# claussss/ubisoft-laforge-daft-exprt

Measured on AMD Instinct MI355X. Metric: mel frames/sec (fwd+bwd), higher is better.
Workload: dtype bf16

## Files before the change

include/daft_exprt_hip.h:

```cpp
#ifndef DAFT_EXPRT_HIP_H
#define DAFT_EXPRT_HIP_H

#include <stdint.h>

#ifdef __cplusplus
extern "C" {
#endif

int dx_version(void);
const char* dx_last_error(void);
int dx_prof_enable(int kind, int capacity);
int dx_prof_collect(int kind, int* launches, double* total_ms);

int dx_int_durations(const float* dur, int B, int L, int sampling_rate, int filter_length, int hop_length, int centered,
                     long long* out, long long* totals, int* status);

int dx_pack_dims(int Cout, int Cin, int bf16, int* dims);
int dx_pack_weights(const float* W, void* fwd, void* bwd, int Cout, int Cin, int taps, int bf16, void* stream);
int dx_pack_weights_batched(const void* descs, int n, int bf16, void* stream);
int dx_pack_weights_host(const void* descs, int n, int bf16, void* stream);
int dx_conv_gemm(const void* X, int ldx, const void* Wp, const float* bias, void* Y, int ldy,
                 int B, int N, int Cin, int Cout, int taps, int bf16,
                 int relu, const float* post_scale, const float* post_shift,
                 const void* relu_aux, int ld_aux, int accumulate,
                 const int* lens, int mask_rows, float out_scale, int skip_halo,
                 int x_bf16, int y_bf16, int aux_bf16, const int* rows_exist, void* stream);
int dx_conv_wgrad(const void* dY, int ldy, const void* X, int ldx, float* G,
                  int B, int N, int Cin, int Cout, int taps, const int* lens, int skip_halo,
                  int bf16, int dy_bf16, int x_bf16, float* dbias, const int* rows_exist, void* stream);
typedef struct DxWgradJob {
  const void* dY; const void* X; float* G; float* dbias; const int* lens;
  int ldy, ldx, B, N, Cin, Cout, skip_halo, reserved;
  const int* rows_exist;
} DxWgradJob;
int dx_conv_wgrad_batched(const void* jobs, int njobs, int taps, int dy_bf16, int x_bf16, void* stream);
int dx_unpack_wgrad(const float* G, float* grad, int Cout, int Cin, int taps, int accumulate, void* stream);
int dx_ff_pair(const void* X, int ldx, const void* Wa, const void* Wb, const float* bias_a, const float* bias_b,
               const void* aux, int ld_aux, void* H, int ldh, float* Y, int ldy,
               int B, int N, int F, int relu_mid, int accumulate, const int* lens, int skip_halo, const int* rows_exist, void* stream);
int dx_ff_pair_ln(const void* X, int ldx, const void* Wa, const void* Wb, const float* bias_a, const float* bias_b, void* H, int ldh, float* Z,
                  int B, int N, int F, const int* lens, int skip_halo, const int* rows_exist,
                  const float* res, const float* ln_w, const float* ln_b, const float* film, int ld_film, float* Yln, float* mean, float* rstd,
                  uint64_t seed_pre, float p_pre, const uint64_t* seed_offset, void* hmask, void* stream);
int dx_ff_pair_ln_qkv(const void* X, int ldx, const void* Wa, const void* Wb, const float* bias_a, const float* bias_b, void* H, int ldh, float* Z,
                      int B, int N, int F, const int* lens, int skip_halo, const int* rows_exist,
                      const float* res, const float* ln_w, const float* ln_b, const float* film, int ld_film, float* Yln, float* mean, float* rstd,
                      uint64_t seed_pre, float p_pre, const uint64_t* seed_offset, const void* Wq, const float* bias_q, void* QKV, void* hmask, void* stream);
int dx_ff_pair_lnbwd(const void* X, int ldx, const void* Wa, const void* Wb, const void* aux, int ld_aux, void* H, int ldh, float* Y,
                     int B, int N, int F, const int* lens, int skip_halo,
                     const float* z, const float* mean, const float* rstd, const float* ln_w, const float* ln_b, void* DG, float* dw, float* db,
                     uint64_t seed_pre, float p_pre, const uint64_t* seed_offset, void* stream);
int dx_ff_block_bwd(const float* dY2, const float* z2, const float* mean2, const float* rstd2, const float* ln2_w, const float* ln2_b,
                    const float* film, int ld_film, void* DG2, float* dw2, float* db2, float* dfilm, int ld_dfilm, uint64_t seed2, float p2,
                    const void* Wa, const void* Wb, const void* aux, int ld_aux, void* H, int ldh, float* Y,
                    int B, int N, int F, const int* lens, int skip_halo,
                    const float* z1, const float* mean1, const float* rstd1, const float* ln1_w, const float* ln1_b, void* DG1, float* dw1, float* db1,
                    uint64_t seed1, float p1, const void* Wout_bwd, void* DATT, const uint64_t* seed_offset, const void* hmask,
                    const int* rows_exist, void* stream);
int dx_colsum(const void* X, int ldx, float* out, long rows, int C, int x_bf16, void* stream);

int dx_length_order(const int* lens, int* order, int B, void* stream);
int dx_attention_fwd(const void* qkv, int ld, const int* lens, void* ctx, int ldc, float* lse,
                     int B, int N, int H, int D, uint64_t seed, const uint64_t* seed_offset, float p_drop, int bf16, int qkv_bf16, int ctx_bf16,
                     const int* order, void* stream);
int dx_attention_proj_ln_fwd(const void* qkv, int ld, const int* lens, void* ctx, int ldc, float* lse, int B, int N, int H, int D,
                             uint64_t seed, const uint64_t* seed_offset, float p_drop,
                             const void* Wpack, const float* proj_bias, float* z, const float* res, const float* w, const float* bias,
                             const float* film, int ld_film, float* y, float* mean, float* rstd, uint64_t seed_pre, float p_pre,
                             void* y_bf16_copy, void* stream);
int dx_attention_bwd(const void* qkv, int ld, const void* ctx, const void* dctx, int ldc, const float* lse, float* delta,
                     const int* lens, void* dqkv, int ldg, int B, int N, int H, int D, uint64_t seed, const uint64_t* seed_offset, float p_drop, int bf16,
                     int qkv_bf16, int dqkv_bf16, int ctx_bf16, const int* order, void* stream);

int dx_ln_fwd(void* a, const void* res, const float* w, const float* bias, const float* film, int ld_film,
              const int* lens, int halo, void* y, float* mean, float* rstd, int B, int N, int C,
              uint64_t seed_pre, float p_pre, uint64_t seed_post, float p_post, const uint64_t* seed_offset, int io_bf16, void* y_bf16_copy,
              void* stream);
int dx_film_affine_fwd(const float* gammas, const float* betas, const float* pm, float* film, int B, int nb, int C, void* stream);
int dx_film_affine_bwd(const void* dfilm_ptrs, const float* gammas, const float* betas, const float* pm, float* dgammas, float* dbetas, float* dpm,
                       int B, int nb, int C, void* stream);
int dx_proj_ln_fwd(const void* X, int ldx, const void* Wpack, const float* proj_bias, float* z, const float* res, const float* w, const float* bias,
                   const float* film, int ld_film, const int* lens, int halo, float* y, float* mean, float* rstd, int B, int N,
                   uint64_t seed_pre, float p_pre, const uint64_t* seed_offset, void* y_bf16_copy, void* stream);
int dx_ln_bwd(const void* dy, const void* z, const float* mean, const float* rstd, const float* w, const float* bias,
              const float* film, int ld_film, const int* lens, int halo, void* dz, void* da, float* dw, float* dbias,
              float* dfilm, int ld_dfilm, int B, int N, int C, int relu_mask,
              uint64_t seed_pre, float p_pre, uint64_t seed_post, float p_post, const uint64_t* seed_offset, int io_bf16, void* dg_bf16_copy,
              void* stream);

int dx_add_pos(const float* x, const long* sym, const float* emb, const float* pe, const int* lens, float* out,
               int B, int N, int D, int pe_rows, void* stream);
int dx_mask_rows(const float* in, const int* lens, float* out, int B, int N, int C, void* stream);
int dx_embedding_bwd(const float* dout, const long* sym, const int* lens, float* demb, int B, int N, int D, void* stream);
int dx_accent_sum(const float* prenet, const float* energy, const float* pitch, const float* we, const float* be,
                  const float* wp, const float* bp, const float* pe, const int* lens, float* out,
                  int B, int N, int D, int pe_rows, void* stream);
int dx_scalar_conv_wgrad(const float* dout, int ldd, const float* rowscale, const float* s0, const float* s1, const int* lens,
                         float* dw0, float* db0, float* dw1, float* db1, int B, int N, int D, void* stream);
int dx_mean_pool(const float* x, const int* lens, float* out, int B, int N, int C, void* stream);
int dx_mean_pool_bwd(const float* dout, const int* lens, float* dx, int B, int N, int C, void* stream);
int dx_transpose(const float* in, float* out, int B, int R, int Cc, int accumulate, void* stream);
int dx_relu_bwd(const float* dy, const float* y, float* out, long n, void* stream);
int dx_channel_affine(const void* x, const float* scale, const float* shift, void* out, long rows, int C, int io_bf16, void* stream);
int dx_l2_normalize(const float* x, float* y, int rows, int C, void* stream);
int dx_cross_entropy(const float* logits, const long* target, float* loss, float* dlogits, int B, int S, void* stream);

int dx_duration_scan(const long* dur_int, float* mu, long* totals, int B, int L, void* stream);
int dx_upsample_prep(const float* enc, const float* dur, const float* energy, const float* pitch,
                     const float* wd, const float* bd, const float* we, const float* be, const float* wp, const float* bp,
                     const float* wr, const float* br, const int* lens, float* xs, float* z, float* sigma,
                     int B, int L, int D, void* stream);
int dx_upsample_fwd(const float* xs, const float* mu, const float* sigma, const int* lens, float* weights, float* xup,
                    int B, int L, int T, int D, void* stream);
int dx_upsample_bwd(const float* dxup, const float* xs, const float* mu, const float* sigma, const float* weights, const int* lens,
                    float* dxs, float* dsigma, int B, int L, int T, int D, void* stream);
int dx_upsample_sym_bwd(const float* dxs_in, const float* dsigma, const float* xs, const float* z, const float* dur, const int* lens,
                        const float* wd, const float* bd, const float* wr, float* dxs_out, float* dz, float* dwr, float* dbr,
                        int B, int L, int D, void* stream);

int dx_mel_stats(const float* mel_pred, const float* mel_target, float* ep, float* et, float* l1sum, float* l2sum,
                 int B, int M, int T, void* stream);
int dx_energy_diff(const float* ep, const float* et, const int* lens, float* des, float* esum, int B, int T, const int* rows_exist, void* stream);
int dx_mel_grad(const float* mel_pred, const float* mel_target, const float* ep, const float* des, const int* lens,
                float c_l1, float c_l2, float c_e, int e_per_total, float* dmel, int B, int M, int T, void* stream);
int dx_loss_finalize(const float* ce, const float* spk_w_dev, float spk_w, const float* dlogits, float* d_spk, int n_logits,
                     const float* pm, float* d_pm, int n_pm, float pmw,
                     const float* l1sum, const float* l2sum, const int* lens, int B, int M, float msw,
                     const float* esum, float ecw, const float* psum, float pcw, float* terms, float* total, float grad_scale, void* stream);
int dx_pitch_mse(const float* pp, int ldp, const float* gt, const int* lens, float* sums, int B, int T, void* stream);
int dx_pitch_grad(const float* pp, int ldp, const float* gt, const int* lens, const float* sums, float scale, float* dpp, int ldd, int B, int T, void* stream);
int dx_pitch_chain_fwd(const float* mel, int B, int M, int T, const int* lens, const void* w0, const void* w1, const void* w2,
                       const float* b0, const float* b1, const float* b2, const float* s0, const float* s1, const float* s2,
                       const float* t0, const float* t1, const float* t2, const float* w3, float b3, float* pp, void* masks,
                       const int* rows_exist, void* stream);
int dx_pitch_chain_bwd(const float* dpp, int B, int M, int T, const int* lens, const void* w0, const void* w1, const void* w2,
                       const float* s0, const float* s1, const float* s2, const float* w3, const void* masks, float* dmel,
                       const int* rows_exist, void* stream);

int dx_condition_prosody(const float* in, float* out, const long* speaker_ids, const float* table, const int* valid,
                         int which, int B, int N, int S, void* stream);
int dx_gather_speaker_rows(const float* emb, const long* speaker_ids, const int* valid, float* out, int B, int E, int S, void* stream);

int dx_sumsq(const float* x, long n, float* out, void* stream);
int dx_adam_step(float* p, const float* g, float* m, float* v, long n, float lr, float beta1, float beta2, float eps,
                 float weight_decay, int step, const float* normsq, float max_norm, float grad_scale, int* skipped,
                 float* norm_out, float* zero_after, void* stream);

#ifdef __cplusplus
}
#endif
#endif
```

ubisoft_laforge_daft_exprt_amd/csrc/dx_attention.hip:

```cpp
#include "dx_common.h"
#include <algorithm>
#include <type_traits>

namespace {

constexpr int HD = 64;
constexpr int TLD = 68;
constexpr float QSCALE = 0.125f;
constexpr bool kSplitBuild = std::is_same<dx_h16, __bf16>::value;
constexpr float LOG2E = 1.4426950408889634f;
constexpr float QSCALE2 = QSCALE * LOG2E;

struct AttnArgs {
  const float* qkv; int ld;
  const int* lens;
  float* ctx; int ldc;
  float* lse;
  int B, N, H, D;
  uint64_t seed; uint32_t thresh; float inv_keep;
  const uint64_t* seed_offset;
  const int* order;
  int xcd_map;
};

__device__ __forceinline__ f32x4 mma4(const float4& a, const float4& b, f32x4 c) {
  c = __builtin_amdgcn_mfma_f32_16x16x4f32(a.x, b.x, c, 0, 0, 0);
  c = __builtin_amdgcn_mfma_f32_16x16x4f32(a.y, b.y, c, 0, 0, 0);
  c = __builtin_amdgcn_mfma_f32_16x16x4f32(a.z, b.z, c, 0, 0, 0);
  c = __builtin_amdgcn_mfma_f32_16x16x4f32(a.w, b.w, c, 0, 0, 0);
  return c;
}

__device__ __forceinline__ void stage_tile(float* dst, const float* base, int ld, int col0, int r0, int N, int tid) {
  for (int u = tid; u < 64 * 16; u += 256) {
    const int row = u >> 4, q = u & 15;
    float4 v = make_float4(0.f, 0.f, 0.f, 0.f);
    if (r0 + row < N) v = *reinterpret_cast<const float4*>(base + (size_t)(r0 + row) * ld + col0 + q * 4);
    *reinterpret_cast<float4*>(dst + row * TLD + q * 4) = v;
  }
}

struct AttnBlock { int tile, h, z; };
__device__ __forceinline__ AttnBlock attn_block(int xcd_map) {
  AttnBlock o{(int)blockIdx.x, (int)blockIdx.y, (int)blockIdx.z};
  if (xcd_map) {
    const int ntx = gridDim.x, H = gridDim.y;
    const int lin = blockIdx.x + ntx * (blockIdx.y + H * blockIdx.z);
    const int xcd = lin & 7, j = lin >> 3;
    const int pair = (j / ntx) * 8 + xcd;
    o.tile = j - (j / ntx) * ntx;
    o.h = pair % H;
    o.z = pair / H;
  }
  return o;
}

__device__ __forceinline__ uint64_t drop_index(int bh, int N, int q, int key) {
  return ((uint64_t)((size_t)bh * N + q) << 16) | (uint64_t)key;
}

__global__ __launch_bounds__(256, 2) void attn_fwd_kernel(const AttnArgs a_) {
  AttnArgs a = a_;
  if (a.seed_offset) a.seed += *a.seed_offset;
  __shared__ __attribute__((aligned(16))) float Ks[64 * TLD];
  __shared__ __attribute__((aligned(16))) float Vs[64 * TLD];
  const AttnBlock blk = attn_block(a.xcd_map);
  const int b = a.order ? a.order[blk.z] : blk.z, h = blk.h, q0 = blk.tile * 64;
  const int tid = threadIdx.x, lane = tid & 63, wave = tid >> 6;
  const int r = lane & 15, g = lane >> 4;
  const int len = a.lens[b];
  const float* base = a.qkv + (size_t)b * a.N * a.ld;
  const int qrow = q0 + wave * 16 + r;
  float* out = a.ctx + ((size_t)b * a.N + qrow) * a.ldc + h * HD;
  if (q0 >= len) {
    if (qrow < a.N) {
#pragma unroll
      for (int dt = 0; dt < 4; ++dt) *reinterpret_cast<float4*>(out + dt * 16 + g * 4) = make_float4(0.f, 0.f, 0.f, 0.f);
      if (g == 0) a.lse[((size_t)b * a.H + h) * a.N + qrow] = 0.f;
    }
    return;
  }
  const int qload = min(qrow, a.N - 1);
  float4 qf[4];
#pragma unroll
  for (int ks = 0; ks < 4; ++ks) {
    const float4 v = *reinterpret_cast<const float4*>(base + (size_t)qload * a.ld + h * HD + ks * 16 + g * 4);
    qf[ks] = make_float4(v.x * QSCALE, v.y * QSCALE, v.z * QSCALE, v.w * QSCALE);
  }
  f32x4 o[4];
#pragma unroll
  for (int dt = 0; dt < 4; ++dt) o[dt] = f32x4{0.f, 0.f, 0.f, 0.f};
  float m_run = -INFINITY, l_run = 0.f;
  const int bh = b * a.H + h;
  const int ntiles = (len + 63) / 64;
  for (int kt0 = 0; kt0 < ntiles; ++kt0) {
    const int kbase = kt0 * 64;
    __syncthreads();
    stage_tile(Ks, base, a.ld, a.D + h * HD, kbase, a.N, tid);
    stage_tile(Vs, base, a.ld, 2 * a.D + h * HD, kbase, a.N, tid);
    __syncthreads();
    f32x4 st[4];
    float mx = -INFINITY;
#pragma unroll
    for (int kt = 0; kt < 4; ++kt) {
      f32x4 acc = f32x4{0.f, 0.f, 0.f, 0.f};
#pragma unroll
      for (int ks = 0; ks < 4; ++ks) {
        const float4 kf = *reinterpret_cast<const float4*>(Ks + (kt * 16 + r) * TLD + ks * 16 + g * 4);
        acc = mma4(kf, qf[ks], acc);
      }
#pragma unroll
      for (int e = 0; e < 4; ++e) {
        if (kbase + kt * 16 + g * 4 + e >= len) acc[e] = -INFINITY;
        mx = fmaxf(mx, acc[e]);
      }
      st[kt] = acc;
    }
    mx = fmaxf(mx, __shfl_xor(mx, 16, 64));
    mx = fmaxf(mx, __shfl_xor(mx, 32, 64));
    const float m_new = fmaxf(m_run, mx);
    const float alpha = expf(m_run - m_new);
    float ls = 0.f;
#pragma unroll
    for (int kt = 0; kt < 4; ++kt) {
      float keep[4] = {1.f, 1.f, 1.f, 1.f};
      if (a.thresh) dx_dropout_scale4(a.seed, drop_index(bh, a.N, qrow, kbase + kt * 16 + g * 4), a.thresh, a.inv_keep, keep);
#pragma unroll
      for (int e = 0; e < 4; ++e) {
        const float p = expf(st[kt][e] - m_new);
        ls += p;
        st[kt][e] = p * keep[e];
      }
    }
    ls += __shfl_xor(ls, 16, 64);
    ls += __shfl_xor(ls, 32, 64);
    l_run = l_run * alpha + ls;
    m_run = m_new;
#pragma unroll
    for (int dt = 0; dt < 4; ++dt) {
      f32x4 acc = o[dt];
#pragma unroll
      for (int e = 0; e < 4; ++e) acc[e] *= alpha;
#pragma unroll
      for (int kt = 0; kt < 4; ++kt) {
#pragma unroll
        for (int e = 0; e < 4; ++e) {
          const float vf = Vs[(kt * 16 + g * 4 + e) * TLD + dt * 16 + r];
          acc = __builtin_amdgcn_mfma_f32_16x16x4f32(vf, st[kt][e], acc, 0, 0, 0);
        }
      }
      o[dt] = acc;
    }
  }
  if (qrow < a.N) {
    const bool valid = qrow < len;
    const float inv = valid ? 1.f / l_run : 0.f;
#pragma unroll
    for (int dt = 0; dt < 4; ++dt)
      *reinterpret_cast<float4*>(out + dt * 16 + g * 4) = make_float4(o[dt][0] * inv, o[dt][1] * inv, o[dt][2] * inv, o[dt][3] * inv);
    if (g == 0) a.lse[((size_t)b * a.H + h) * a.N + qrow] = valid ? m_run + logf(l_run) : 0.f;
  }
}

__global__ __launch_bounds__(256) void attn_delta_kernel(const float* __restrict__ dctx, const float* __restrict__ ctx, int ldc,
                                                         float* __restrict__ delta, int B, int N, int H) {
  const int lane = threadIdx.x & 63;
  const long items = (long)B * N * H;
  for (long it = (long)blockIdx.x * 4 + (threadIdx.x >> 6); it < items; it += (long)gridDim.x * 4) {
    const int h = (int)(it % H);
    const long row = it / H;
    const int b = (int)(row / N), n = (int)(row - (long)b * N);
    const float v = dctx[row * ldc + h * HD + lane] * ctx[row * ldc + h * HD + lane];
    const float s = dx_wave_sum(v);
    if (lane == 0) delta[((size_t)b * H + h) * N + n] = s;
  }
}

struct AttnBwdArgs {
  const float* qkv; int ld;
  const float* dctx; int ldc;
  const float* lse; const float* delta;
  const int* lens;
  float* dqkv; int ldg;
  int B, N, H, D;
  uint64_t seed; uint32_t thresh; float inv_keep;
  const float* ctx;
  float* delta_out;
  const uint64_t* seed_offset;
  const int* order;
  int xcd_map;
};

__global__ __launch_bounds__(256, 2) void attn_bwd_dq_kernel(const AttnBwdArgs a_) {
  AttnBwdArgs a = a_;
  if (a.seed_offset) a.seed += *a.seed_offset;
  __shared__ __attribute__((aligned(16))) float Ks[64 * TLD];
  __shared__ __attribute__((aligned(16))) float Vs[64 * TLD];
  const AttnBlock blk = attn_block(a.xcd_map);
  const int b = a.order ? a.order[blk.z] : blk.z, h = blk.h, q0 = blk.tile * 64;
  const int tid = threadIdx.x, lane = tid & 63, wave = tid >> 6;
  const int r = lane & 15, g = lane >> 4;
  const int len = a.lens[b];
  const float* base = a.qkv + (size_t)b * a.N * a.ld;
  const int qrow = q0 + wave * 16 + r;
  float* out = a.dqkv + ((size_t)b * a.N + qrow) * a.ldg + h * HD;
  if (q0 >= len) {
    if (qrow < a.N) {
#pragma unroll
      for (int dt = 0; dt < 4; ++dt) *reinterpret_cast<float4*>(out + dt * 16 + g * 4) = make_float4(0.f, 0.f, 0.f, 0.f);
    }
    return;
  }
  const int qload = min(qrow, a.N - 1);
  const int bh = b * a.H + h;
  float4 qf[4], gf[4];
#pragma unroll
  for (int ks = 0; ks < 4; ++ks) {
    const float4 v = *reinterpret_cast<const float4*>(base + (size_t)qload * a.ld + h * HD + ks * 16 + g * 4);
    qf[ks] = make_float4(v.x * QSCALE, v.y * QSCALE, v.z * QSCALE, v.w * QSCALE);
    gf[ks] = *reinterpret_cast<const float4*>(a.dctx + ((size_t)b * a.N + qload) * a.ldc + h * HD + ks * 16 + g * 4);
  }
  const float lse_q = a.lse[(size_t)bh * a.N + qload];
  const float delta_q = a.delta[(size_t)bh * a.N + qload];
  f32x4 dq[4];
#pragma unroll
  for (int dt = 0; dt < 4; ++dt) dq[dt] = f32x4{0.f, 0.f, 0.f, 0.f};
  const int ntiles = (len + 63) / 64;
  for (int kt0 = 0; kt0 < ntiles; ++kt0) {
    const int kbase = kt0 * 64;
    __syncthreads();
    stage_tile(Ks, base, a.ld, a.D + h * HD, kbase, a.N, tid);
    stage_tile(Vs, base, a.ld, 2 * a.D + h * HD, kbase, a.N, tid);
    __syncthreads();
    f32x4 ds[4];
#pragma unroll
    for (int kt = 0; kt < 4; ++kt) {
      f32x4 s = f32x4{0.f, 0.f, 0.f, 0.f}, dp = f32x4{0.f, 0.f, 0.f, 0.f};
#pragma unroll
      for (int ks = 0; ks < 4; ++ks) {
        const float4 kf = *reinterpret_cast<const float4*>(Ks + (kt * 16 + r) * TLD + ks * 16 + g * 4);
        const float4 vf = *reinterpret_cast<const float4*>(Vs + (kt * 16 + r) * TLD + ks * 16 + g * 4);
        s = mma4(kf, qf[ks], s);
        dp = mma4(vf, gf[ks], dp);
      }
      float keep[4] = {1.f, 1.f, 1.f, 1.f};
      if (a.thresh) dx_dropout_scale4(a.seed, drop_index(bh, a.N, qrow, kbase + kt * 16 + g * 4), a.thresh, a.inv_keep, keep);
#pragma unroll
      for (int e = 0; e < 4; ++e) {
        const bool masked = kbase + kt * 16 + g * 4 + e >= len;
        const float p = masked ? 0.f : expf(s[e] - lse_q);
        s[e] = p * (dp[e] * keep[e] - delta_q) * QSCALE;
      }
      ds[kt] = s;
    }
#pragma unroll
    for (int dt = 0; dt < 4; ++dt) {
      f32x4 acc = dq[dt];
#pragma unroll
      for (int kt = 0; kt < 4; ++kt) {
#pragma unroll
        for (int e = 0; e < 4; ++e) {
          const float kf = Ks[(kt * 16 + g * 4 + e) * TLD + dt * 16 + r];
          acc = __builtin_amdgcn_mfma_f32_16x16x4f32(kf, ds[kt][e], acc, 0, 0, 0);
        }
      }
      dq[dt] = acc;
    }
  }
  if (qrow < a.N) {
    const float z = qrow < len ? 1.f : 0.f;
#pragma unroll
    for (int dt = 0; dt < 4; ++dt)
      *reinterpret_cast<float4*>(out + dt * 16 + g * 4) = make_float4(dq[dt][0] * z, dq[dt][1] * z, dq[dt][2] * z, dq[dt][3] * z);
  }
}

__global__ __launch_bounds__(256, 2) void attn_bwd_dkv_kernel(const AttnBwdArgs a_) {
  AttnBwdArgs a = a_;
  if (a.seed_offset) a.seed += *a.seed_offset;
  __shared__ __attribute__((aligned(16))) float Qs[64 * TLD];
  __shared__ __attribute__((aligned(16))) float Gs[64 * TLD];
  __shared__ float lse_s[64], delta_s[64];
  const AttnBlock blk = attn_block(a.xcd_map);
  const int b = a.order ? a.order[blk.z] : blk.z, h = blk.h, k0 = blk.tile * 64;
  const int tid = threadIdx.x, lane = tid & 63, wave = tid >> 6;
  const int r = lane & 15, g = lane >> 4;
  const int len = a.lens[b];
  const float* base = a.qkv + (size_t)b * a.N * a.ld;
  const float* gbase = a.dctx + (size_t)b * a.N * a.ldc;
  const int krow = k0 + wave * 16 + r;
  float* outk = a.dqkv + ((size_t)b * a.N + krow) * a.ldg + a.D + h * HD;
  float* outv = a.dqkv + ((size_t)b * a.N + krow) * a.ldg + 2 * a.D + h * HD;
  if (k0 >= len) {
    if (krow < a.N) {
#pragma unroll
      for (int dt = 0; dt < 4; ++dt) {
        *reinterpret_cast<float4*>(outk + dt * 16 + g * 4) = make_float4(0.f, 0.f, 0.f, 0.f);
        *reinterpret_cast<float4*>(outv + dt * 16 + g * 4) = make_float4(0.f, 0.f, 0.f, 0.f);
      }
    }
    return;
  }
  const int kload = min(krow, a.N - 1);
  const bool key_valid = krow < len;
  const int bh = b * a.H + h;
  float4 kf[4], vf[4];
#pragma unroll
  for (int ks = 0; ks < 4; ++ks) {
    const float4 v = *reinterpret_cast<const float4*>(base + (size_t)kload * a.ld + a.D + h * HD + ks * 16 + g * 4);
    kf[ks] = make_float4(v.x * QSCALE, v.y * QSCALE, v.z * QSCALE, v.w * QSCALE);
    vf[ks] = *reinterpret_cast<const float4*>(base + (size_t)kload * a.ld + 2 * a.D + h * HD + ks * 16 + g * 4);
  }
  f32x4 dk[4], dv[4];
#pragma unroll
  for (int dt = 0; dt < 4; ++dt) { dk[dt] = f32x4{0.f, 0.f, 0.f, 0.f}; dv[dt] = f32x4{0.f, 0.f, 0.f, 0.f}; }
  const int ntiles = (len + 63) / 64;
  for (int qt0 = 0; qt0 < ntiles; ++qt0) {
    const int qbase = qt0 * 64;
    __syncthreads();
    stage_tile(Qs, base, a.ld, h * HD, qbase, a.N, tid);
    stage_tile(Gs, gbase, a.ldc, h * HD, qbase, a.N, tid);
    if (tid < 64) {
      const int q = qbase + tid;
      lse_s[tid] = q < a.N ? a.lse[(size_t)bh * a.N + q] : 0.f;
      delta_s[tid] = q < a.N ? a.delta[(size_t)bh * a.N + q] : 0.f;
    }
    __syncthreads();
    f32x4 pd[4], ds[4];
#pragma unroll
    for (int qt = 0; qt < 4; ++qt) {
      f32x4 s = f32x4{0.f, 0.f, 0.f, 0.f}, dp = f32x4{0.f, 0.f, 0.f, 0.f};
#pragma unroll
      for (int ks = 0; ks < 4; ++ks) {
        const float4 qf = *reinterpret_cast<const float4*>(Qs + (qt * 16 + r) * TLD + ks * 16 + g * 4);
        const float4 gf = *reinterpret_cast<const float4*>(Gs + (qt * 16 + r) * TLD + ks * 16 + g * 4);
        s = mma4(qf, kf[ks], s);
        dp = mma4(gf, vf[ks], dp);
      }
#pragma unroll
      for (int e = 0; e < 4; ++e) {
        const int ql = qt * 16 + g * 4 + e, q = qbase + ql;
        const bool live = key_valid && q < len;
        const float p = live ? expf(s[e] - lse_s[ql]) : 0.f;
// ... 279 lines not shown
#pragma unroll
  for (int dt = 0; dt < 4; ++dt) { dk[dt] = f32x4{0.f, 0.f, 0.f, 0.f}; dv[dt] = f32x4{0.f, 0.f, 0.f, 0.f}; }
  const int ntiles = (len + 63) / 64;
  for (int qt0 = 0; qt0 < ntiles; ++qt0) {
    const int qbase = qt0 * 64;
    __syncthreads();
    stage_split<true, true>(Qh, Ql, Qth, Qtl, base, a.ld, h * HD, qbase, a.N, tid);
    stage_split<true, true>(Gh, Gl, Gth, Gtl, gbase, a.ldc, h * HD, qbase, a.N, tid);
    if (tid < 64) {
      const int q = qbase + tid;
      lse_s[tid] = q < a.N ? a.lse[(size_t)bh * a.N + q] : 0.f;
      delta_s[tid] = q < a.N ? a.delta[(size_t)bh * a.N + q] : 0.f;
    }
    __syncthreads();
    f32x4 pd[4], ds[4];
#pragma unroll
    for (int qt = 0; qt < 4; ++qt) {
      f32x4 s = f32x4{0.f, 0.f, 0.f, 0.f}, dp = f32x4{0.f, 0.f, 0.f, 0.f};
#pragma unroll
      for (int c = 0; c < 2; ++c) {
        s = dx_mma_split3(split_frag(Qh, qt * 16 + r, c, g), split_frag(Ql, qt * 16 + r, c, g), kh[c], kl[c], s);
        dp = dx_mma_split3(split_frag(Gh, qt * 16 + r, c, g), split_frag(Gl, qt * 16 + r, c, g), vh[c], vl[c], dp);
      }
#pragma unroll
      for (int e = 0; e < 4; ++e) {
        const int ql_ = qt * 16 + g * 4 + e, q = qbase + ql_;
        const bool live = key_valid && q < len;
        const float p = live ? expf(s[e] - lse_s[ql_]) : 0.f;
        float keep = 1.f;
        if (a.thresh) keep = dx_dropout_scale(a.seed, drop_index(bh, a.N, q, krow), a.thresh, a.inv_keep);
        pd[qt][e] = p * keep;
        ds[qt][e] = p * (dp[e] * keep - delta_s[ql_]) * QSCALE;
      }
    }
    dx_bf16x8 ph[2], pl[2], dh[2], dl[2];
#pragma unroll
    for (int c = 0; c < 2; ++c) { split_bf16x8(pd[2 * c], pd[2 * c + 1], ph[c], pl[c]); split_bf16x8(ds[2 * c], ds[2 * c + 1], dh[c], dl[c]); }
#pragma unroll
    for (int dt = 0; dt < 4; ++dt) {
#pragma unroll
      for (int c = 0; c < 2; ++c) {
        dv[dt] = dx_mma_split3(split_frag(Gth, dt * 16 + r, c, g), split_frag(Gtl, dt * 16 + r, c, g), ph[c], pl[c], dv[dt]);
        dk[dt] = dx_mma_split3(split_frag(Qth, dt * 16 + r, c, g), split_frag(Qtl, dt * 16 + r, c, g), dh[c], dl[c], dk[dt]);
      }
    }
  }
  if (krow < a.N) {
#pragma unroll
    for (int dt = 0; dt < 4; ++dt) {
      *reinterpret_cast<float4*>(outk + dt * 16 + g * 4) = make_float4(dk[dt][0], dk[dt][1], dk[dt][2], dk[dt][3]);
      *reinterpret_cast<float4*>(outv + dt * 16 + g * 4) = make_float4(dv[dt][0], dv[dt][1], dv[dt][2], dv[dt][3]);
    }
  }
}


typedef short s16x4 __attribute__((ext_vector_type(4)));
typedef short s16x8 __attribute__((ext_vector_type(8)));

__device__ __forceinline__ int sw_off(int row, int slot) { return row * 128 + ((slot ^ (row & 7)) << 4); }

#include "dx_rowvec.h"

__device__ __forceinline__ void stage_tile_bf16(unsigned char* dst, const float* base, int ld, int col0, int r0, int N, int tid, float scale) {
#pragma unroll
  for (int it = 0; it < 4; ++it) {
    const int u = tid + it * 256;
    const int row = u >> 4, q = u & 15;
    float4 v = make_float4(0.f, 0.f, 0.f, 0.f);
    if (r0 + row < N) v = *reinterpret_cast<const float4*>(base + (size_t)(r0 + row) * ld + col0 + q * 4);
    bf16x4 h;
    h[0] = (dx_h16)(v.x * scale); h[1] = (dx_h16)(v.y * scale); h[2] = (dx_h16)(v.z * scale); h[3] = (dx_h16)(v.w * scale);
    *reinterpret_cast<uint2*>(dst + sw_off(row, q >> 1) + ((q & 1) << 3)) = __builtin_bit_cast(uint2, h);
  }
}

#define DX_TILE_LOAD(QT_, REG, BASE, LD, COL0, R0, NROWS)                                                         \
  if constexpr (sizeof(QT_) == 4) {                                                                               \
    _Pragma("unroll") for (int it = 0; it < 4; ++it) {                                                           \
      const int u_ = tid + it * 256;                                                                              \
      const int row_ = u_ >> 4, q_ = u_ & 15;                                                                     \
      f32x4 v_ = f32x4{0.f, 0.f, 0.f, 0.f};                                                                       \
      if ((R0) + row_ < (NROWS)) v_ = *reinterpret_cast<const f32x4*>((BASE) + (size_t)((R0) + row_) * (LD) + (COL0) + q_ * 4); \
      REG[it] = v_;                                                                                               \
    }                                                                                                             \
  } else {                                                                                                        \
    _Pragma("unroll") for (int it = 0; it < 2; ++it) {                                                           \
      const int u_ = tid + it * 256;                                                                              \
      const int row_ = u_ >> 3, q_ = u_ & 7;                                                                      \
      f32x4 v_ = f32x4{0.f, 0.f, 0.f, 0.f};                                                                       \
      if ((R0) + row_ < (NROWS)) v_ = *reinterpret_cast<const f32x4*>((BASE) + (size_t)((R0) + row_) * (LD) + (COL0) + q_ * 8); \
      REG[it] = v_;                                                                                               \
    }                                                                                                             \
  }
#define DX_TILE_STORE(QT_, REG, DST)                                                                              \
  if constexpr (sizeof(QT_) == 4) {                                                                               \
    _Pragma("unroll") for (int it = 0; it < 4; ++it) {                                                           \
      const int u_ = tid + it * 256;                                                                              \
      const int row_ = u_ >> 4, q_ = u_ & 15;                                                                     \
      bf16x4 h_;                                                                                                  \
      h_[0] = (dx_h16)REG[it][0]; h_[1] = (dx_h16)REG[it][1]; h_[2] = (dx_h16)REG[it][2]; h_[3] = (dx_h16)REG[it][3]; \
      *reinterpret_cast<uint2*>((DST) + sw_off(row_, q_ >> 1) + ((q_ & 1) << 3)) = __builtin_bit_cast(uint2, h_); \
    }                                                                                                             \
  } else {                                                                                                        \
    _Pragma("unroll") for (int it = 0; it < 2; ++it) {                                                           \
      const int u_ = tid + it * 256;                                                                              \
      *reinterpret_cast<f32x4*>((DST) + sw_off(u_ >> 3, u_ & 7)) = REG[it];                                       \
    }                                                                                                             \
  }

__device__ __forceinline__ bf16x8 row_frag(const unsigned char* tile, int row, int ks, int g) {
  return __builtin_bit_cast(bf16x8, *reinterpret_cast<const float4*>(tile + sw_off(row, ks * 4 + g)));
}

__device__ __forceinline__ s16x4 tr_half(const unsigned char* tile, int row0, int col0, int lane) {
  const int li = lane & 15, q = li >> 2, p = li & 3;
  const unsigned char* addr = tile + sw_off(row0 + q, (col0 >> 3) + (p >> 1)) + ((p & 1) << 3);
  return __builtin_amdgcn_ds_read_tr16_b64_v4i16((__attribute__((address_space(3))) s16x4*)(addr));
}
__device__ __forceinline__ bf16x8 tr_pair(const unsigned char* tile, int rowA, int rowB, int col0, int lane) {
  const s16x4 lo = tr_half(tile, rowA, col0, lane), hi = tr_half(tile, rowB, col0, lane);
  const s16x8 v = {lo[0], lo[1], lo[2], lo[3], hi[0], hi[1], hi[2], hi[3]};
  return __builtin_bit_cast(bf16x8, v);
}
__device__ __forceinline__ bf16x8 pack_pair(const f32x4& a, const f32x4& b) {
  bf16x8 h;
  h[0] = (dx_h16)a[0]; h[1] = (dx_h16)a[1]; h[2] = (dx_h16)a[2]; h[3] = (dx_h16)a[3];
  h[4] = (dx_h16)b[0]; h[5] = (dx_h16)b[1]; h[6] = (dx_h16)b[2]; h[7] = (dx_h16)b[3];
  return h;
}
__device__ __forceinline__ bf16x8 load_row8(const float* p, float scale) {
  const float4 a = *reinterpret_cast<const float4*>(p), b = *reinterpret_cast<const float4*>(p + 4);
  bf16x8 h;
  h[0] = (dx_h16)(a.x * scale); h[1] = (dx_h16)(a.y * scale); h[2] = (dx_h16)(a.z * scale); h[3] = (dx_h16)(a.w * scale);
  h[4] = (dx_h16)(b.x * scale); h[5] = (dx_h16)(b.y * scale); h[6] = (dx_h16)(b.z * scale); h[7] = (dx_h16)(b.w * scale);
  return h;
}
__device__ __forceinline__ bf16x8 load_row8(const dx_h16* p, float scale) {
  bf16x8 h = *reinterpret_cast<const bf16x8*>(p);
  if (scale != 1.f) {
#pragma unroll
    for (int e = 0; e < 8; ++e) h[e] = (dx_h16)((float)h[e] * scale);
  }
  return h;
}
__device__ __forceinline__ void store4(float* p, float a, float b, float c, float d) { *reinterpret_cast<float4*>(p) = make_float4(a, b, c, d); }
__device__ __forceinline__ void store4(dx_h16* p, float a, float b, float c, float d) {
  bf16x4 h; h[0] = (dx_h16)a; h[1] = (dx_h16)b; h[2] = (dx_h16)c; h[3] = (dx_h16)d;
  *reinterpret_cast<bf16x4*>(p) = h;
}
#define DX_MFMA_BF16(A, B, C) DX_MFMA_H16((A), (B), (C))
__device__ __forceinline__ float dx_max2(float a, float b) { return __builtin_amdgcn_fmed3f(a, b, INFINITY); }

template <typename QT, typename CT>
__global__ __launch_bounds__(256, 2) void attn_fwd_bf16_kernel(const AttnArgs a_) {
  AttnArgs a = a_;
  if (a.seed_offset) a.seed += *a.seed_offset;
  __shared__ __attribute__((aligned(16))) unsigned char Ks[64 * 128];
  __shared__ __attribute__((aligned(16))) unsigned char Vs[64 * 128];
  const AttnBlock blk = attn_block(a.xcd_map);
  const int b = a.order ? a.order[blk.z] : blk.z, h = blk.h, q0 = blk.tile * 64;
  const int tid = threadIdx.x, lane = tid & 63, wave = tid >> 6;
  const int r = lane & 15, g = lane >> 4;
  const int len = a.lens[b];
  const QT* base = reinterpret_cast<const QT*>(a.qkv) + (size_t)b * a.N * a.ld;
  const int qrow = q0 + wave * 16 + r;
  CT* out = reinterpret_cast<CT*>(a.ctx) + ((size_t)b * a.N + qrow) * a.ldc + h * HD;
  if (q0 >= len) {
    if (qrow < a.N) {
#pragma unroll
      for (int dt = 0; dt < 4; ++dt) store4(out + dt * 16 + g * 4, 0.f, 0.f, 0.f, 0.f);
      if (g == 0) a.lse[((size_t)b * a.H + h) * a.N + qrow] = 0.f;
    }
    return;
  }
  const int qload = min(qrow, a.N - 1);
  bf16x8 qf[2];
#pragma unroll
  for (int ks = 0; ks < 2; ++ks) qf[ks] = load_row8(base + (size_t)qload * a.ld + h * HD + ks * 32 + g * 8, QSCALE2);
  f32x4 o[4];
#pragma unroll
  for (int dt = 0; dt < 4; ++dt) o[dt] = f32x4{0.f, 0.f, 0.f, 0.f};
  float m_run = -INFINITY, l_run = 0.f;
  const int bh = b * a.H + h;
  const int ntiles = (len + 63) / 64;
  const uint64_t drow = (uint64_t)((size_t)bh * a.N + qrow) << 14;
  const uint32_t thresh_v = a.thresh;
  f32x4 kreg[4], vreg[4];
  DX_TILE_LOAD(QT, kreg, base, a.ld, a.D + h * HD, 0, a.N)
  DX_TILE_LOAD(QT, vreg, base, a.ld, 2 * a.D + h * HD, 0, a.N)
  for (int kt0 = 0; kt0 < ntiles; ++kt0) {
    const int kbase = kt0 * 64;
    __syncthreads();
    DX_TILE_STORE(QT, kreg, Ks)
    DX_TILE_STORE(QT, vreg, Vs)
    __syncthreads();
    if (kt0 + 1 < ntiles) {
      DX_TILE_LOAD(QT, kreg, base, a.ld, a.D + h * HD, kbase + 64, a.N)
      DX_TILE_LOAD(QT, vreg, base, a.ld, 2 * a.D + h * HD, kbase + 64, a.N)
    }
    f32x4 st[4];
    float mx = -INFINITY;
    const bool tail_tile = kbase + 64 > len;
#pragma unroll
    for (int kt = 0; kt < 4; ++kt) {
      f32x4 acc = f32x4{0.f, 0.f, 0.f, 0.f};
#pragma unroll
      for (int ks = 0; ks < 2; ++ks) acc = DX_MFMA_BF16(row_frag(Ks, kt * 16 + r, ks, g), qf[ks], acc);
      if (tail_tile) {
#pragma unroll
        for (int e = 0; e < 4; ++e)
          if (kbase + kt * 16 + g * 4 + e >= len) acc[e] = -INFINITY;
      }
      mx = dx_max2(mx, dx_max2(dx_max2(acc[0], acc[1]), dx_max2(acc[2], acc[3])));
      st[kt] = acc;
    }
    mx = dx_max2(mx, __shfl_xor(mx, 16, 64));
    mx = dx_max2(mx, __shfl_xor(mx, 32, 64));
    const float m_new = dx_max2(m_run, mx);
    const bool rescale = __builtin_amdgcn_ballot_w64(m_new > m_run) != 0;
    float ls = 0.f;
#pragma unroll
    for (int kt = 0; kt < 4; ++kt) {
      float pk[4];
#pragma unroll
      for (int e = 0; e < 4; ++e) {
        pk[e] = __builtin_amdgcn_exp2f(st[kt][e] - m_new);
        ls += pk[e];
      }
      if (a.thresh) dx_keep4(dx_rand64(a.seed, drow | (uint64_t)((kbase + kt * 16 + g * 4) >> 2)), thresh_v, pk, 0.f);
#pragma unroll
      for (int e = 0; e < 4; ++e) st[kt][e] = pk[e];
    }
    ls += __shfl_xor(ls, 16, 64);
    ls += __shfl_xor(ls, 32, 64);
    if (rescale) {
      const float alpha = __builtin_amdgcn_exp2f(m_run - m_new);
      l_run *= alpha;
#pragma unroll
      for (int dt = 0; dt < 4; ++dt)
#pragma unroll
        for (int e = 0; e < 4; ++e) o[dt][e] *= alpha;
    }
    l_run += ls;
    m_run = m_new;
    const bf16x8 p01 = pack_pair(st[0], st[1]), p23 = pack_pair(st[2], st[3]);
#pragma unroll
    for (int dt = 0; dt < 4; ++dt) {
      f32x4 acc = o[dt];
      acc = DX_MFMA_BF16(tr_pair(Vs, 0 + g * 4, 16 + g * 4, dt * 16, lane), p01, acc);
      acc = DX_MFMA_BF16(tr_pair(Vs, 32 + g * 4, 48 + g * 4, dt * 16, lane), p23, acc);
      o[dt] = acc;
    }
  }
  if (qrow < a.N) {
    const bool valid = qrow < len;
    const float inv = valid ? (a.thresh ? a.inv_keep : 1.f) / l_run : 0.f;
#pragma unroll
    for (int dt = 0; dt < 4; ++dt) store4(out + dt * 16 + g * 4, o[dt][0] * inv, o[dt][1] * inv, o[dt][2] * inv, o[dt][3] * inv);
    if (g == 0) a.lse[((size_t)b * a.H + h) * a.N + qrow] = valid ? m_run + __log2f(l_run) : 0.f;
  }
}

constexpr float APL_LN_EPS = 1e-5f;
struct AttnProjLnArgs {
  AttnArgs at;
  const dx_h16* Wp; const float* proj_bias;
  float* z; const float* res; const float* w; const float* bias;
  const float* film; int ld_film;
  float* y; dx_h16* y_h; float* mean; float* rstd;
  uint64_t seed_pre; uint32_t thresh_pre; float inv_keep_pre;
};

__global__ __launch_bounds__(512, 4) void attn_proj_ln_fwd_kernel(const AttnProjLnArgs p_) {
  typedef dx_h16 QT;
  typedef dx_h16 CT;
  constexpr int C = 128;
  AttnArgs a = p_.at;
  uint64_t seed_pre = p_.seed_pre;
  if (a.seed_offset) { const uint64_t o = *a.seed_offset; a.seed += o; seed_pre += o; }
  __shared__ __attribute__((aligned(16))) unsigned char smem[4 * 64 * 128 + 64 * 256];
  const int tid512 = threadIdx.x, lane = tid512 & 63;
  const int wave = __builtin_amdgcn_readfirstlane(tid512 >> 6);
  const int h = wave >> 2, wq = wave & 3;
  const int tid = tid512 & 255;
  unsigned char* const Ks = smem + h * (64 * 128);
  unsigned char* const Vs = smem + 2 * 64 * 128 + h * (64 * 128);
  unsigned char* const Cs = smem + 4 * 64 * 128;
  float* const tile = reinterpret_cast<float*>(smem);
  const int r = lane & 15, g = lane >> 4;
  const int ntx = (a.N + 63) / 64;
  const int xcd = blockIdx.x & 7, j = blockIdx.x >> 3;
  const int b = (j / ntx) * 8 + xcd, q0 = (j - (j / ntx) * ntx) * 64;
  if (b >= a.B) return;
  const int len = a.lens[b];
  const QT* base = reinterpret_cast<const QT*>(a.qkv) + (size_t)b * a.N * a.ld;
  const int qrow = q0 + wq * 16 + r;
  CT* out = reinterpret_cast<CT*>(a.ctx) + ((size_t)b * a.N + qrow) * a.ldc + h * HD;
  constexpr int E = RowVec<C>::E, LPR = RowVec<C>::LPR;
  const int l = lane % LPR, sub = lane / LPR;
  if (q0 >= len) {
    if (qrow < a.N) {
#pragma unroll
      for (int dt = 0; dt < 4; ++dt) store4(out + dt * 16 + g * 4, 0.f, 0.f, 0.f, 0.f);
      if (g == 0) a.lse[((size_t)b * a.H + h) * a.N + qrow] = 0.f;
    }
    float zero[E];
#pragma unroll
    for (int e = 0; e < E; ++e) zero[e] = 0.f;
#pragma unroll
    for (int st = 0; st < 2; ++st) {
      const int n = q0 + wave * 8 + st * 4 + sub;
      if (n < a.N) {
        const long row = (long)b * a.N + n;
        row_store<C>(p_.z + row * C, l, zero);
        row_store<C>(p_.y + row * C, l, zero);
        if (p_.y_h) row_store<C>(p_.y_h + row * C, l, zero);
        if (l == 0) { p_.mean[row] = 0.f; p_.rstd[row] = 0.f; }
      }
    }
    return;
  }
  const int qload = min(qrow, a.N - 1);
  bf16x8 qf[2];
#pragma unroll
  for (int ks = 0; ks < 2; ++ks) qf[ks] = load_row8(base + (size_t)qload * a.ld + h * HD + ks * 32 + g * 8, QSCALE2);
  f32x4 o[4];
#pragma unroll
  for (int dt = 0; dt < 4; ++dt) o[dt] = f32x4{0.f, 0.f, 0.f, 0.f};
  float m_run = -INFINITY, l_run = 0.f;
  const int bh = b * a.H + h;
  const int ntiles = (len + 63) / 64;
  const uint64_t drow = (uint64_t)((size_t)bh * a.N + qrow) << 14;
  const uint32_t thresh_v = a.thresh;
  f32x4 kreg[4], vreg[4];
  DX_TILE_LOAD(QT, kreg, base, a.ld, a.D + h * HD, 0, a.N)
  DX_TILE_LOAD(QT, vreg, base, a.ld, 2 * a.D + h * HD, 0, a.N)
  for (int kt0 = 0; kt0 < ntiles; ++kt0) {
    const int kbase = kt0 * 64;
    __syncthreads();
    DX_TILE_STORE(QT, kreg, Ks)
    DX_TILE_STORE(QT, vreg, Vs)
    __syncthreads();
    if (kt0 + 1 < ntiles) {
      DX_TILE_LOAD(QT, kreg, base, a.ld, a.D + h * HD, kbase + 64, a.N)
      DX_TILE_LOAD(QT, vreg, base, a.ld, 2 * a.D + h * HD, kbase + 64, a.N)
    }
    f32x4 st[4];
    float mx = -INFINITY;
    const bool tail_tile = kbase + 64 > len;
#pragma unroll
    for (int kt = 0; kt < 4; ++kt) {
      f32x4 acc = f32x4{0.f, 0.f, 0.f, 0.f};
#pragma unroll
      for (int ks = 0; ks < 2; ++ks) acc = DX_MFMA_BF16(row_frag(Ks, kt * 16 + r, ks, g), qf[ks], acc);
      if (tail_tile) {
#pragma unroll
        for (int e = 0; e < 4; ++e)
          if (kbase + kt * 16 + g * 4 + e >= len) acc[e] = -INFINITY;
      }
      mx = dx_max2(mx, dx_max2(dx_max2(acc[0], acc[1]), dx_max2(acc[2], acc[3])));
      st[kt] = acc;
    }
    mx = dx_max2(mx, __shfl_xor(mx, 16, 64));
    mx = dx_max2(mx, __shfl_xor(mx, 32, 64));
    const float m_new = dx_max2(m_run, mx);
    const bool rescale = __builtin_amdgcn_ballot_w64(m_new > m_run) != 0;
    float ls = 0.f;
#pragma unroll
    for (int kt = 0; kt < 4; ++kt) {
      float pk[4];
#pragma unroll
      for (int e = 0; e < 4; ++e) {
        pk[e] = __builtin_amdgcn_exp2f(st[kt][e] - m_new);
        ls += pk[e];
      }
      if (a.thresh) dx_keep4(dx_rand64(a.seed, drow | (uint64_t)((kbase + kt * 16 + g * 4) >> 2)), thresh_v, pk, 0.f);
#pragma unroll
      for (int e = 0; e < 4; ++e) st[kt][e] = pk[e];
    }
    ls += __shfl_xor(ls, 16, 64);
    ls += __shfl_xor(ls, 32, 64);
    if (rescale) {
      const float alpha = __builtin_amdgcn_exp2f(m_run - m_new);
      l_run *= alpha;
#pragma unroll
      for (int dt = 0; dt < 4; ++dt)
#pragma unroll
        for (int e = 0; e < 4; ++e) o[dt][e] *= alpha;
    }
    l_run += ls;
    m_run = m_new;
    const bf16x8 p01 = pack_pair(st[0], st[1]), p23 = pack_pair(st[2], st[3]);
#pragma unroll
    for (int dt = 0; dt < 4; ++dt) {
      f32x4 acc = o[dt];
      acc = DX_MFMA_BF16(tr_pair(Vs, 0 + g * 4, 16 + g * 4, dt * 16, lane), p01, acc);
      acc = DX_MFMA_BF16(tr_pair(Vs, 32 + g * 4, 48 + g * 4, dt * 16, lane), p23, acc);
      o[dt] = acc;
    }
  }
  {
    const bool valid = qrow < len;
    const float inv = valid ? (a.thresh ? a.inv_keep : 1.f) / l_run : 0.f;
    const int crow = wq * 16 + r;
#pragma unroll
    for (int dt = 0; dt < 4; ++dt) {
      bf16x4 c4;
      c4[0] = (dx_h16)(o[dt][0] * inv); c4[1] = (dx_h16)(o[dt][1] * inv); c4[2] = (dx_h16)(o[dt][2] * inv); c4[3] = (dx_h16)(o[dt][3] * inv);
      if (qrow < a.N) *reinterpret_cast<bf16x4*>(out + dt * 16 + g * 4) = c4;
      const int slot = h * 8 + dt * 2 + (g >> 1);
      *reinterpret_cast<bf16x4*>(Cs + crow * 256 + ((slot ^ (crow & 15)) << 4) + ((g & 1) << 3)) = c4;
    }
    if (qrow < a.N && g == 0) a.lse[((size_t)b * a.H + h) * a.N + qrow] = valid ? m_run + __log2f(l_run) : 0.f;
  }
  bool valid[2]; long rown[2];
  float rv[2][E];
#pragma unroll
  for (int st = 0; st < 2; ++st) {
    const int n = q0 + wave * 8 + st * 4 + sub;
    const bool inb = n < a.N;
    valid[st] = inb && n < len;
    rown[st] = inb ? (long)b * a.N + n : -1;
#pragma unroll
    for (int e = 0; e < E; ++e) rv[st][e] = 0.f;
    if (valid[st] && p_.res) row_load<C>(p_.res + rown[st] * C, l, rv[st]);
  }
  float wv[E], bv[E];
#pragma unroll
  for (int e = 0; e < E; ++e) { wv[e] = p_.w[row_col<C>(l, e)]; bv[e] = p_.bias[row_col<C>(l, e)]; }
  __syncthreads();
  {
    const int tok = wq * 16 + r;
    const bool live = q0 + tok < len;
    if (__builtin_amdgcn_ballot_w64(live) != 0) {
      bf16x8 xb[4];
#pragma unroll
      for (int ks = 0; ks < 4; ++ks) xb[ks] = *reinterpret_cast<const bf16x8*>(Cs + tok * 256 + (((ks * 4 + g) ^ (tok & 15)) << 4));
      f32x4 acc[4];
#pragma unroll
      for (int i = 0; i < 4; ++i)
        acc[i] = p_.proj_bias ? *reinterpret_cast<const f32x4*>(p_.proj_bias + (h * 4 + i) * 16 + g * 4) : f32x4{0.f, 0.f, 0.f, 0.f};
#pragma unroll
      for (int ks = 0; ks < 4; ++ks) {
        bf16x8 wa[4];
#pragma unroll
        for (int i = 0; i < 4; ++i) wa[i] = *reinterpret_cast<const bf16x8*>(p_.Wp + (size_t)((h * 4 + i) * 4 + ks) * 512 + lane * 8);
#pragma unroll
        for (int i = 0; i < 4; ++i) acc[i] = DX_MFMA_H16(wa[i], xb[ks], acc[i]);
      }
#pragma unroll
      for (int i = 0; i < 4; ++i)
        *reinterpret_cast<f32x4*>(tile + tok * C + ((((h * 4 + i) * 4 + g) ^ (tok & 15)) << 2)) = acc[i];
    }
  }
  __syncthreads();
#pragma unroll
  for (int st = 0; st < 2; ++st) {
    const int lrow = wave * 8 + st * 4 + sub;
    const long row = rown[st];
    const bool inb = row >= 0, vld = valid[st];
    float z[E];
#pragma unroll
    for (int e = 0; e < E; ++e) z[e] = 0.f;
    if (vld) {
#pragma unroll
      for (int k = 0; k < RowVec<C>::K; ++k) {
        const f32x4 t = *reinterpret_cast<const f32x4*>(tile + lrow * C + (((k * LPR + l) ^ (lrow & 15)) << 2));
        z[k * 4 + 0] = t[0]; z[k * 4 + 1] = t[1]; z[k * 4 + 2] = t[2]; z[k * 4 + 3] = t[3];
      }
      if (p_.thresh_pre) {
        float f[E];
        row_dropout<C>(seed_pre, (uint64_t)row, l, p_.thresh_pre, p_.inv_keep_pre, f);
#pragma unroll
        for (int e = 0; e < E; ++e) z[e] *= f[e];
      }
#pragma unroll
      for (int e = 0; e < E; ++e) z[e] += rv[st][e];
    }
    if (inb) row_store<C>(p_.z + row * C, l, z);
    float s = 0.f;
#pragma unroll
    for (int e = 0; e < E; ++e) s += z[e];
    const float mu = row_sum<C>(s) * (1.0f / C);
    float q = 0.f;
#pragma unroll
    for (int e = 0; e < E; ++e) { const float d = z[e] - mu; q += d * d; }
    const float rs = 1.0f / sqrtf(row_sum<C>(q) * (1.0f / C) + APL_LN_EPS);
    if (inb && l == 0) { p_.mean[row] = vld ? mu : 0.f; p_.rstd[row] = vld ? rs : 0.f; }
    float y[E];
#pragma unroll
    for (int e = 0; e < E; ++e) {
      const int c = row_col<C>(l, e);
      float t = (z[e] - mu) * rs * wv[e] + bv[e];
      if (p_.film) t = p_.film[(size_t)b * p_.ld_film + c] * t + p_.film[(size_t)b * p_.ld_film + C + c];
      y[e] = vld ? t : 0.f;
    }
    if (inb) {
      row_store<C>(p_.y + row * C, l, y);
      if (p_.y_h) row_store<C>(p_.y_h + row * C, l, y);
    }
  }
}

__device__ __forceinline__ void load8f(const float* p, float v[8]) {
  const float4 a = *reinterpret_cast<const float4*>(p), b = *reinterpret_cast<const float4*>(p + 4);
  v[0] = a.x; v[1] = a.y; v[2] = a.z; v[3] = a.w; v[4] = b.x; v[5] = b.y; v[6] = b.z; v[7] = b.w;
}
__device__ __forceinline__ void load8f(const dx_h16* p, float v[8]) {
  const bf16x8 h = *reinterpret_cast<const bf16x8*>(p);
#pragma unroll
  for (int e = 0; e < 8; ++e) v[e] = (float)h[e];
}

template <typename QT, typename OT, typename CT>
__global__ __launch_bounds__(256, 2) void attn_bwd_dq_bf16_kernel(const AttnBwdArgs a_) {
  AttnBwdArgs a = a_;
  if (a.seed_offset) a.seed += *a.seed_offset;
  __shared__ __attribute__((aligned(16))) unsigned char Ks[64 * 128];
  __shared__ __attribute__((aligned(16))) unsigned char Vs[64 * 128];
  const AttnBlock blk = attn_block(a.xcd_map);
  const int b = a.order ? a.order[blk.z] : blk.z, h = blk.h, q0 = blk.tile * 64;
  const int tid = threadIdx.x, lane = tid & 63, wave = tid >> 6;
  const int r = lane & 15, g = lane >> 4;
  const int len = a.lens[b];
  const QT* base = reinterpret_cast<const QT*>(a.qkv) + (size_t)b * a.N * a.ld;
  const int qrow = q0 + wave * 16 + r;
  OT* out = reinterpret_cast<OT*>(a.dqkv) + ((size_t)b * a.N + qrow) * a.ldg + h * HD;
  if (q0 >= len) {
    if (qrow < a.N) {
#pragma unroll
      for (int dt = 0; dt < 4; ++dt) store4(out + dt * 16 + g * 4, 0.f, 0.f, 0.f, 0.f);
    }
    return;
  }
  const int qload = min(qrow, a.N - 1);
  const int bh = b * a.H + h;
  bf16x8 qf[2], gf[2];
  float delta_q = 0.f;
  const float ik = a.thresh ? a.inv_keep : 1.f;
#pragma unroll
  for (int ks = 0; ks < 2; ++ks) {
    qf[ks] = load_row8(base + (size_t)qload * a.ld + h * HD + ks * 32 + g * 8, QSCALE2);
    const size_t o = ((size_t)b * a.N + qload) * a.ldc + h * HD + ks * 32 + g * 8;
    float gv[8], cv[8];
    load8f(reinterpret_cast<const CT*>(a.dctx) + o, gv);
    load8f(reinterpret_cast<const CT*>(a.ctx) + o, cv);
    bf16x8 hg;
#pragma unroll
    for (int e = 0; e < 8; ++e) hg[e] = (dx_h16)(gv[e] * ik);
    gf[ks] = hg;
    delta_q += (gv[0] * cv[0] + gv[1] * cv[1]) + (gv[2] * cv[2] + gv[3] * cv[3]) + (gv[4] * cv[4] + gv[5] * cv[5]) + (gv[6] * cv[6] + gv[7] * cv[7]);
  }
  delta_q += __shfl_xor(delta_q, 16, 64);
  delta_q += __shfl_xor(delta_q, 32, 64);
  if (g == 0 && qrow < a.N) a.delta_out[(size_t)bh * a.N + qrow] = delta_q;
  const float lse_q = a.lse[(size_t)bh * a.N + qload];
  const float neg_delta_q = -delta_q;
  const f32x4 neg_lse4 = f32x4{-lse_q, -lse_q, -lse_q, -lse_q};
  f32x4 dq[4];
#pragma unroll
  for (int dt = 0; dt < 4; ++dt) dq[dt] = f32x4{0.f, 0.f, 0.f, 0.f};
  const int ntiles = (len + 63) / 64;
  const uint64_t drow = (uint64_t)((size_t)bh * a.N + qrow) << 14;
  const uint32_t thresh_v = a.thresh;
  f32x4 kreg[4], vreg[4];
  DX_TILE_LOAD(QT, kreg, base, a.ld, a.D + h * HD, 0, a.N)
  DX_TILE_LOAD(QT, vreg, base, a.ld, 2 * a.D + h * HD, 0, a.N)
  for (int kt0 = 0; kt0 < ntiles; ++kt0) {
    const int kbase = kt0 * 64;
    __syncthreads();
    DX_TILE_STORE(QT, kreg, Ks)
    DX_TILE_STORE(QT, vreg, Vs)
    __syncthreads();
    if (kt0 + 1 < ntiles) {
      DX_TILE_LOAD(QT, kreg, base, a.ld, a.D + h * HD, kbase + 64, a.N)
      DX_TILE_LOAD(QT, vreg, base, a.ld, 2 * a.D + h * HD, kbase + 64, a.N)
    }
    f32x4 ds[4];
    const bool tail_tile = kbase + 64 > len;
#pragma unroll
    for (int kt = 0; kt < 4; ++kt) {
      f32x4 s = neg_lse4, dp = f32x4{0.f, 0.f, 0.f, 0.f};
#pragma unroll
      for (int ks = 0; ks < 2; ++ks) {
        s = DX_MFMA_BF16(row_frag(Ks, kt * 16 + r, ks, g), qf[ks], s);
        dp = DX_MFMA_BF16(row_frag(Vs, kt * 16 + r, ks, g), gf[ks], dp);
      }
      float u[4] = {dp[0] - delta_q, dp[1] - delta_q, dp[2] - delta_q, dp[3] - delta_q};
      if (a.thresh) dx_keep4(dx_rand64(a.seed, drow | (uint64_t)((kbase + kt * 16 + g * 4) >> 2)), thresh_v, u, neg_delta_q);
      float p[4];
#pragma unroll
      for (int e = 0; e < 4; ++e) p[e] = __builtin_amdgcn_exp2f(s[e]);
      if (tail_tile) {
#pragma unroll
        for (int e = 0; e < 4; ++e)
          if (kbase + kt * 16 + g * 4 + e >= len) p[e] = 0.f;
      }
#pragma unroll
      for (int e = 0; e < 4; ++e) s[e] = p[e] * u[e];
      ds[kt] = s;
    }
    const bf16x8 d01 = pack_pair(ds[0], ds[1]), d23 = pack_pair(ds[2], ds[3]);
#pragma unroll
    for (int dt = 0; dt < 4; ++dt) {
      f32x4 acc = dq[dt];
      acc = DX_MFMA_BF16(tr_pair(Ks, 0 + g * 4, 16 + g * 4, dt * 16, lane), d01, acc);
      acc = DX_MFMA_BF16(tr_pair(Ks, 32 + g * 4, 48 + g * 4, dt * 16, lane), d23, acc);
      dq[dt] = acc;
    }
  }
  if (qrow < a.N) {
    const float z = qrow < len ? QSCALE : 0.f;
#pragma unroll
    for (int dt = 0; dt < 4; ++dt)
      store4(out + dt * 16 + g * 4, dq[dt][0] * z, dq[dt][1] * z, dq[dt][2] * z, dq[dt][3] * z);
  }
}

template <typename QT, typename OT, typename CT>
__global__ __launch_bounds__(256, (sizeof(QT) == 2 && sizeof(CT) == 2) ? 3 : 2) void attn_bwd_dkv_bf16_kernel(const AttnBwdArgs a_) {
  AttnBwdArgs a = a_;
  if (a.seed_offset) a.seed += *a.seed_offset;
  __shared__ __attribute__((aligned(16))) unsigned char Qs[64 * 128];
  __shared__ __attribute__((aligned(16))) unsigned char Gs[64 * 128];
  __shared__ __attribute__((aligned(16))) float lse_s[64], delta_s[64];
  const AttnBlock blk = attn_block(a.xcd_map);
  const int b = a.order ? a.order[blk.z] : blk.z, h = blk.h, k0 = blk.tile * 64;
  const int tid = threadIdx.x, lane = tid & 63, wave = tid >> 6;
  const int r = lane & 15, g = lane >> 4;
  const int len = a.lens[b];
  const QT* base = reinterpret_cast<const QT*>(a.qkv) + (size_t)b * a.N * a.ld;
  const CT* gbase = reinterpret_cast<const CT*>(a.dctx) + (size_t)b * a.N * a.ldc;
  const int krow = k0 + wave * 16 + r;
  OT* outk = reinterpret_cast<OT*>(a.dqkv) + ((size_t)b * a.N + krow) * a.ldg + a.D + h * HD;
  OT* outv = reinterpret_cast<OT*>(a.dqkv) + ((size_t)b * a.N + krow) * a.ldg + 2 * a.D + h * HD;
  if (k0 >= len) {
    if (krow < a.N) {
#pragma unroll
      for (int dt = 0; dt < 4; ++dt) {
        store4(outk + dt * 16 + g * 4, 0.f, 0.f, 0.f, 0.f);
        store4(outv + dt * 16 + g * 4, 0.f, 0.f, 0.f, 0.f);
      }
    }
    return;
  }
  const int kload = min(krow, a.N - 1);
  const bool key_valid = krow < len;
  const int bh = b * a.H + h;
  bf16x8 kf[2], vf[2];
#pragma unroll
  for (int ks = 0; ks < 2; ++ks) {
    kf[ks] = load_row8(base + (size_t)kload * a.ld + a.D + h * HD + ks * 32 + g * 8, QSCALE2);
    vf[ks] = load_row8(base + (size_t)kload * a.ld + 2 * a.D + h * HD + ks * 32 + g * 8, a.thresh ? a.inv_keep : 1.f);
  }
  const uint32_t fsel = 0x0c0c0000u | (uint32_t)((2 * (krow & 3) + 1) << 8) | (uint32_t)(2 * (krow & 3));
  const uint32_t thresh_v = a.thresh;
  f32x4 dk[4], dv[4];
#pragma unroll
  for (int dt = 0; dt < 4; ++dt) { dk[dt] = f32x4{0.f, 0.f, 0.f, 0.f}; dv[dt] = f32x4{0.f, 0.f, 0.f, 0.f}; }
  const int ntiles = (len + 63) / 64;
  f32x4 qreg[4], greg[4];
  float lse_r = 0.f, delta_r = 0.f;
  DX_TILE_LOAD(QT, qreg, base, a.ld, h * HD, 0, a.N)
  DX_TILE_LOAD(CT, greg, gbase, a.ldc, h * HD, 0, a.N)
  if (tid < 64 && tid < a.N) { lse_r = a.lse[(size_t)bh * a.N + tid]; delta_r = a.delta[(size_t)bh * a.N + tid]; }
  for (int qt0 = 0; qt0 < ntiles; ++qt0) {
    const int qbase = qt0 * 64;
    __syncthreads();
    DX_TILE_STORE(QT, qreg, Qs)
    DX_TILE_STORE(CT, greg, Gs)
    if (tid < 64) { lse_s[tid] = -lse_r; delta_s[tid] = delta_r; }
    __syncthreads();
    if (qt0 + 1 < ntiles) {
      DX_TILE_LOAD(QT, qreg, base, a.ld, h * HD, qbase + 64, a.N)
      DX_TILE_LOAD(CT, greg, gbase, a.ldc, h * HD, qbase + 64, a.N)
      const int qn = qbase + 64 + tid;
      lse_r = (tid < 64 && qn < a.N) ? a.lse[(size_t)bh * a.N + qn] : 0.f;
      delta_r = (tid < 64 && qn < a.N) ? a.delta[(size_t)bh * a.N + qn] : 0.f;
    }
    const bool tail_q = qbase + 64 > len, tail_k = k0 + 64 > len;
#pragma unroll
    for (int half = 0; half < 2; ++half) {
      f32x4 pd[2], ds[2];
#pragma unroll
      for (int q2 = 0; q2 < 2; ++q2) {
        const int qt = half * 2 + q2;
        uint32_t wlo = 0, whi = 0;
        if (a.thresh) {
          const uint64_t w = dx_rand64(a.seed, drop_index(bh, a.N, qbase + qt * 16 + g * 4 + (r & 3), krow) >> 2);
          wlo = (uint32_t)w; whi = (uint32_t)(w >> 32);
        }
        f32x4 s = *reinterpret_cast<const f32x4*>(&lse_s[qt * 16 + g * 4]), dp = f32x4{0.f, 0.f, 0.f, 0.f};
#pragma unroll
        for (int ks = 0; ks < 2; ++ks) {
          s = DX_MFMA_BF16(row_frag(Qs, qt * 16 + r, ks, g), kf[ks], s);
          dp = DX_MFMA_BF16(row_frag(Gs, qt * 16 + r, ks, g), vf[ks], dp);
        }
        float p[4];
#pragma unroll
        for (int e = 0; e < 4; ++e) p[e] = __builtin_amdgcn_exp2f(s[e]);
        if (tail_k || tail_q) {
#pragma unroll
          for (int e = 0; e < 4; ++e)
            if (!key_valid || qbase + qt * 16 + g * 4 + e >= len) p[e] = 0.f;
        }
        float pk[4] = {p[0], p[1], p[2], p[3]}, u[4], nd[4];
#pragma unroll
        for (int e = 0; e < 4; ++e) { nd[e] = -delta_s[qt * 16 + g * 4 + e]; u[e] = dp[e] + nd[e]; }
        if (a.thresh) {
          const uint32_t lo0 = __builtin_amdgcn_mov_dpp(wlo, 0x00, 0xF, 0xF, true), hi0 = __builtin_amdgcn_mov_dpp(whi, 0x00, 0xF, 0xF, true);
          const uint32_t lo1 = __builtin_amdgcn_mov_dpp(wlo, 0x55, 0xF, 0xF, true), hi1 = __builtin_amdgcn_mov_dpp(whi, 0x55, 0xF, 0xF, true);
          const uint32_t lo2 = __builtin_amdgcn_mov_dpp(wlo, 0xAA, 0xF, 0xF, true), hi2 = __builtin_amdgcn_mov_dpp(whi, 0xAA, 0xF, 0xF, true);
          const uint32_t lo3 = __builtin_amdgcn_mov_dpp(wlo, 0xFF, 0xF, 0xF, true), hi3 = __builtin_amdgcn_mov_dpp(whi, 0xFF, 0xF, 0xF, true);
          const uint32_t lo[4] = {lo0, lo1, lo2, lo3}, hi[4] = {hi0, hi1, hi2, hi3};
#pragma unroll
          for (int e = 0; e < 4; ++e)
            dx_keep2(__builtin_amdgcn_perm(hi[e], lo[e], fsel), thresh_v, pk[e], u[e], nd[e]);
        }
#pragma unroll
        for (int e = 0; e < 4; ++e) {
          pd[q2][e] = pk[e];
          ds[q2][e] = p[e] * u[e];
        }
      }
      const bf16x8 pp = pack_pair(pd[0], pd[1]), dd = pack_pair(ds[0], ds[1]);
#pragma unroll
      for (int dt = 0; dt < 4; ++dt) {
        dv[dt] = DX_MFMA_BF16(tr_pair(Gs, half * 32 + g * 4, half * 32 + 16 + g * 4, dt * 16, lane), pp, dv[dt]);
        dk[dt] = DX_MFMA_BF16(tr_pair(Qs, half * 32 + g * 4, half * 32 + 16 + g * 4, dt * 16, lane), dd, dk[dt]);
      }
    }
  }
  if (krow < a.N) {
#pragma unroll
    for (int dt = 0; dt < 4; ++dt) {
      store4(outk + dt * 16 + g * 4, dk[dt][0] * QSCALE, dk[dt][1] * QSCALE, dk[dt][2] * QSCALE, dk[dt][3] * QSCALE);
      const float ik = a.thresh ? a.inv_keep : 1.f;
      store4(outv + dt * 16 + g * 4, dv[dt][0] * ik, dv[dt][1] * ik, dv[dt][2] * ik, dv[dt][3] * ik);
    }
  }
}
#undef DX_MFMA_BF16
#undef DX_TILE_LOAD
#undef DX_TILE_STORE

__global__ __launch_bounds__(1024) void length_order_kernel(const int* __restrict__ lens, int* __restrict__ order, int B) {
  __shared__ int ls[1024];
  const int t = threadIdx.x;
  if (t < B) ls[t] = lens[t];
  __syncthreads();
  if (t >= B) return;
  const int mine = ls[t];
  int rank = 0;
  for (int j = 0; j < B; ++j) rank += (ls[j] > mine) || (ls[j] == mine && j < t);
  order[rank] = t;
}

int check_common(const char* who, const void* qkv, int ld, int B, int N, int H, int D) {
  DX_REQUIRE(qkv != nullptr, "%s: null pointer", who);
  DX_REQUIRE(B > 0 && N > 0 && H > 0 && D == H * HD, "%s: head dim must be 64 (D=%d, H=%d)", who, D, H);
  DX_REQUIRE(ld >= 3 * D && (ld % 4) == 0 && ((uintptr_t)qkv % 16) == 0, "%s: qkv must be 16-byte aligned with ld >= 3*D, ld %% 4 == 0", who);
  DX_REQUIRE(N < 65536, "%s: sequence length %d too long", who, N);
  return DX_OK;
}

}

extern "C" {

int dx_length_order(const int* lens, int* order, int B, void* stream) {
  DX_REQUIRE(lens && order && B > 0 && B <= 1024, "dx_length_order: bad arguments (B <= 1024)");
  hipLaunchKernelGGL(length_order_kernel, dim3(1), dim3(1024), 0, (hipStream_t)stream, lens, order, B);
  DX_LAUNCH_CHECK("dx_length_order");
  return DX_OK;
}

int dx_attention_fwd(const void* qkvv, int ld, const int* lens, void* ctxv, int ldc, float* lse,
                     int B, int N, int H, int D, uint64_t seed, const uint64_t* seed_offset, float p_drop, int bf16, int qkv_bf16, int ctx_bf16,
                     const int* order, void* stream) {
  float* ctx = (float*)ctxv;
  const float* qkv = (const float*)qkvv;
  if (int rc = check_common("dx_attention_fwd", qkv, ld, B, N, H, D)) return rc;
  DX_REQUIRE(bf16 == 0 || bf16 == 1 || (bf16 == 2 && kSplitBuild), "dx_attention_fwd: bad operand mode %d", bf16);
  const bool split = bf16 == 2;
  if (split) bf16 = 0;
  DX_REQUIRE(!qkv_bf16 || (bf16 && (ld % 8) == 0), "dx_attention_fwd: bf16-stored qkv needs bf16 mode and ld %% 8 == 0");
  DX_REQUIRE(lens && ctx && lse && ldc >= D && (ldc % 4) == 0 && ((uintptr_t)ctx % 16) == 0, "dx_attention_fwd: bad output arguments");
  DX_REQUIRE(!ctx_bf16 || (bf16 && (ldc % 8) == 0), "dx_attention_fwd: a 16-bit context needs the 16-bit operand mode and ldc %% 8 == 0");
  DX_REQUIRE(p_drop >= 0.f && p_drop < 1.f, "dx_attention_fwd: dropout p out of range");
  AttnArgs a{qkv, ld, lens, ctx, ldc, lse, B, N, H, D, seed, (uint32_t)lrintf(p_drop * 65536.f), 1.f / (1.f - p_drop), seed_offset, order, 0};
  a.xcd_map = (H * B) % 8 == 0;
  hipStream_t s = (hipStream_t)stream;
  dx_prof_begin(DX_PROF_ATTN_FWD, s);
  const dim3 grid(dx_cdiv(N, 64), H, B);
  if (bf16 && qkv_bf16 && ctx_bf16) hipLaunchKernelGGL((attn_fwd_bf16_kernel<dx_h16, dx_h16>), grid, dim3(256), 0, s, a);
  else if (bf16 && qkv_bf16) hipLaunchKernelGGL((attn_fwd_bf16_kernel<dx_h16, float>), grid, dim3(256), 0, s, a);
  else if (bf16 && ctx_bf16) hipLaunchKernelGGL((attn_fwd_bf16_kernel<float, dx_h16>), grid, dim3(256), 0, s, a);
  else if (bf16) hipLaunchKernelGGL((attn_fwd_bf16_kernel<float, float>), grid, dim3(256), 0, s, a);
  else if (split) { if constexpr (kSplitBuild) hipLaunchKernelGGL(attn_fwd_split_kernel, grid, dim3(256), 0, s, a); }
  else hipLaunchKernelGGL(attn_fwd_kernel, dim3(dx_cdiv(N, 64), H, B), dim3(256), 0, s, a);
  dx_prof_end(DX_PROF_ATTN_FWD, s);
  DX_LAUNCH_CHECK("dx_attention_fwd");
  return DX_OK;
}

int dx_attention_proj_ln_fwd(const void* qkv, int ld, const int* lens, void* ctx, int ldc, float* lse, int B, int N, int H, int D,
                             uint64_t seed, const uint64_t* seed_offset, float p_drop,
                             const void* Wpack, const float* proj_bias, float* z, const float* res, const float* w, const float* bias,
                             const float* film, int ld_film, float* y, float* mean, float* rstd, uint64_t seed_pre, float p_pre,
                             void* y_bf16_copy, void* stream) {
  if (int rc = check_common("dx_attention_proj_ln_fwd", qkv, ld, B, N, H, D)) return rc;
  DX_REQUIRE(H == 2 && D == 128 && (ld % 8) == 0 && (ldc % 8) == 0 && ldc >= D, "dx_attention_proj_ln_fwd: 2 heads x 64, 16-bit rows (ld, ldc multiples of 8)");
  DX_REQUIRE(lens && ctx && lse && Wpack && z && w && bias && y && mean && rstd, "dx_attention_proj_ln_fwd: null pointer");
  DX_REQUIRE(((uintptr_t)ctx % 16) == 0 && ((uintptr_t)Wpack % 16) == 0 && ((uintptr_t)z % 16) == 0 && ((uintptr_t)y % 16) == 0 &&
             (!res || ((uintptr_t)res % 16) == 0), "dx_attention_proj_ln_fwd: pointers must be 16-byte aligned");
  DX_REQUIRE(p_drop >= 0.f && p_drop < 1.f && p_pre >= 0.f && p_pre < 1.f, "dx_attention_proj_ln_fwd: dropout p out of range");
  DX_REQUIRE(!film || ld_film >= 256, "dx_attention_proj_ln_fwd: ld_film too small");
  AttnProjLnArgs k{};
  k.at = AttnArgs{(const float*)qkv, ld, lens, (float*)ctx, ldc, lse, B, N, H, D, seed, (uint32_t)lrintf(p_drop * 65536.f), 1.f / (1.f - p_drop), seed_offset, nullptr, 0};
  k.Wp = (const dx_h16*)Wpack; k.proj_bias = proj_bias; k.z = z; k.res = res; k.w = w; k.bias = bias; k.film = film; k.ld_film = ld_film;
  k.y = y; k.y_h = (dx_h16*)y_bf16_copy; k.mean = mean; k.rstd = rstd;
  k.seed_pre = seed_pre; k.thresh_pre = (uint32_t)lrintf(p_pre * 65536.f); k.inv_keep_pre = 1.f / (1.f - p_pre);
  hipStream_t s = (hipStream_t)stream;
  dx_prof_begin(DX_PROF_ATTN_FWD, s);
  hipLaunchKernelGGL(attn_proj_ln_fwd_kernel, dim3(8 * dx_cdiv(N, 64) * dx_cdiv(B, 8)), dim3(512), 0, s, k);
  dx_prof_end(DX_PROF_ATTN_FWD, s);
  DX_LAUNCH_CHECK("dx_attention_proj_ln_fwd");
  return DX_OK;
}

int dx_attention_bwd(const void* qkvv, int ld, const void* ctxv, const void* dctxv, int ldc, const float* lse, float* delta,
                     const int* lens, void* dqkvv, int ldg, int B, int N, int H, int D, uint64_t seed, const uint64_t* seed_offset, float p_drop, int bf16,
                     int qkv_bf16, int dqkv_bf16, int ctx_bf16, const int* order, void* stream) {
  const float* qkv = (const float*)qkvv; float* dqkv = (float*)dqkvv; const float* ctx = (const float*)ctxv; const float* dctx = (const float*)dctxv;
  DX_REQUIRE(bf16 == 0 || bf16 == 1 || (bf16 == 2 && kSplitBuild), "dx_attention_bwd: bad operand mode %d", bf16);
  const bool split = bf16 == 2;
  if (split) bf16 = 0;
  DX_REQUIRE(!ctx_bf16 || (bf16 && (ldc % 8) == 0), "dx_attention_bwd: a 16-bit context needs the 16-bit operand mode and ldc %% 8 == 0");
  if (int rc = check_common("dx_attention_bwd", qkv, ld, B, N, H, D)) return rc;
  DX_REQUIRE(!(qkv_bf16 || dqkv_bf16) || (bf16 && (ld % 8) == 0 && (ldg % 8) == 0), "dx_attention_bwd: bf16-stored qkv/dqkv need bf16 mode and ld %% 8 == 0");
  DX_REQUIRE(ctx && dctx && lse && delta && lens && dqkv, "dx_attention_bwd: null pointer");
  DX_REQUIRE(ldc >= D && (ldc % 4) == 0 && ldg >= 3 * D && (ldg % 4) == 0, "dx_attention_bwd: bad leading dimensions");
  DX_REQUIRE(((uintptr_t)dctx % 16) == 0 && ((uintptr_t)dqkv % 16) == 0, "dx_attention_bwd: pointers must be 16-byte aligned");
  DX_REQUIRE(p_drop >= 0.f && p_drop < 1.f, "dx_attention_bwd: dropout p out of range");
  hipStream_t s = (hipStream_t)stream;
  const long items = (long)B * N * H;
  if (!bf16)
    hipLaunchKernelGGL(attn_delta_kernel, dim3((int)std::min<long>((items + 3) / 4, 8192)), dim3(256), 0, s, dctx, ctx, ldc, delta, B, N, H);
  AttnBwdArgs a{qkv, ld, dctx, ldc, lse, delta, lens, dqkv, ldg, B, N, H, D, seed, (uint32_t)lrintf(p_drop * 65536.f), 1.f / (1.f - p_drop), ctx, delta, seed_offset, order, 0};
  a.xcd_map = (H * B) % 8 == 0;
  dx_prof_begin(DX_PROF_ATTN_BWD, s);
  if (bf16) {
    const dim3 grid(dx_cdiv(N, 64), H, B);
#define DX_ATTN_BWD(QT_, OT_)                                                                          \
    if (ctx_bf16) {                                                                                    \
      hipLaunchKernelGGL((attn_bwd_dq_bf16_kernel<QT_, OT_, dx_h16>), grid, dim3(256), 0, s, a);       \
      hipLaunchKernelGGL((attn_bwd_dkv_bf16_kernel<QT_, OT_, dx_h16>), grid, dim3(256), 0, s, a);      \
    } else {                                                                                           \
      hipLaunchKernelGGL((attn_bwd_dq_bf16_kernel<QT_, OT_, float>), grid, dim3(256), 0, s, a);        \
      hipLaunchKernelGGL((attn_bwd_dkv_bf16_kernel<QT_, OT_, float>), grid, dim3(256), 0, s, a);       \
    }
    if (qkv_bf16 && dqkv_bf16) { DX_ATTN_BWD(dx_h16, dx_h16) }
    else if (qkv_bf16) { DX_ATTN_BWD(dx_h16, float) }
    else if (dqkv_bf16) { DX_ATTN_BWD(float, dx_h16) }
    else { DX_ATTN_BWD(float, float) }
#undef DX_ATTN_BWD
  } else if (split) {
    if constexpr (kSplitBuild) {
      static bool configured = false;
      if (!configured) {
        hipFuncSetAttribute(reinterpret_cast<const void*>(&attn_bwd_dkv_split_kernel), hipFuncAttributeMaxDynamicSharedMemorySize, (int)DKV_SPLIT_SMEM);
        configured = true;
      }
      hipLaunchKernelGGL(attn_bwd_dq_split_kernel, dim3(dx_cdiv(N, 64), H, B), dim3(256), 0, s, a);
      hipLaunchKernelGGL(attn_bwd_dkv_split_kernel, dim3(dx_cdiv(N, 64), H, B), dim3(256), DKV_SPLIT_SMEM, s, a);
    }
  } else {
    hipLaunchKernelGGL(attn_bwd_dq_kernel, dim3(dx_cdiv(N, 64), H, B), dim3(256), 0, s, a);
    hipLaunchKernelGGL(attn_bwd_dkv_kernel, dim3(dx_cdiv(N, 64), H, B), dim3(256), 0, s, a);
  }
  dx_prof_end(DX_PROF_ATTN_BWD, s);
  DX_LAUNCH_CHECK("dx_attention_bwd");
  return DX_OK;
}

}
```

ubisoft_laforge_daft_exprt_amd/csrc/dx_common.h:

```cpp
#pragma once
#include <hip/hip_runtime.h>
#include <stdint.h>
#include <stdio.h>

#define DX_OK 0
#define DX_ERR_ARG 1
#define DX_ERR_LAUNCH 2

#ifdef __cplusplus
extern "C" {
#endif
void dx_set_error(const char* fmt, ...);
void dx_prof_begin(int kernel_id, hipStream_t s);
void dx_prof_end(int kernel_id, hipStream_t s);
#ifdef __cplusplus
}
#endif

#define DX_REQUIRE(cond, ...)              \
  do {                                     \
    if (!(cond)) {                         \
      dx_set_error(__VA_ARGS__);           \
      return DX_ERR_ARG;                   \
    }                                      \
  } while (0)

#define DX_LAUNCH_CHECK(name)                                         \
  do {                                                                \
    hipError_t e_ = hipGetLastError();                                \
    if (e_ != hipSuccess) {                                           \
      dx_set_error("%s: launch failed: %s", name, hipGetErrorString(e_)); \
      return DX_ERR_LAUNCH;                                           \
    }                                                                 \
  } while (0)

enum { DX_PROF_CONV_GEMM = 0, DX_PROF_WGRAD_GEMM = 1, DX_PROF_ATTN_FWD = 2, DX_PROF_ATTN_BWD = 3,
       DX_PROF_UPSAMPLE = 4, DX_PROF_ROWS = 5, DX_PROF_NKINDS = 6 };

typedef float f32x4 __attribute__((ext_vector_type(4)));
#ifdef DX_F16
typedef _Float16 dx_h16;
#define DX_MFMA_H16(A, B, C) __builtin_amdgcn_mfma_f32_16x16x32_f16((A), (B), (C), 0, 0, 0)
#include "dx_f16_names.h"
#else
typedef __bf16 dx_h16;
#define DX_MFMA_H16(A, B, C) __builtin_amdgcn_mfma_f32_16x16x32_bf16((A), (B), (C), 0, 0, 0)
#endif
typedef dx_h16 bf16x8 __attribute__((ext_vector_type(8)));
typedef dx_h16 bf16x4 __attribute__((ext_vector_type(4)));

static inline int dx_cdiv(int a, int b) { return (a + b - 1) / b; }
static inline int dx_roundup(int a, int b) { return dx_cdiv(a, b) * b; }

#ifdef __HIPCC__
typedef __bf16 dx_bf16x8 __attribute__((ext_vector_type(8)));
typedef __bf16 dx_bf16x2 __attribute__((ext_vector_type(2)));
__device__ __forceinline__ void split_bf16x2(float x0, float x1, unsigned& hi, unsigned& lo) {
  dx_bf16x2 h, l;
  h[0] = (__bf16)x0; h[1] = (__bf16)x1;
  const float h0 = (float)h[0], h1 = (float)h[1];
  l[0] = (__bf16)(__builtin_isfinite(h0) ? x0 - h0 : 0.f);
  l[1] = (__bf16)(__builtin_isfinite(h1) ? x1 - h1 : 0.f);
  hi = __builtin_bit_cast(unsigned, h); lo = __builtin_bit_cast(unsigned, l);
}
__device__ __forceinline__ void split_bf16x4(const f32x4& v, uint2& hi, uint2& lo) {
  split_bf16x2(v[0], v[1], hi.x, lo.x);
  split_bf16x2(v[2], v[3], hi.y, lo.y);
}
__device__ __forceinline__ void split_bf16x8(const f32x4& a, const f32x4& b, dx_bf16x8& hi, dx_bf16x8& lo) {
  uint2 ha, la, hb, lb;
  split_bf16x4(a, ha, la);
  split_bf16x4(b, hb, lb);
  hi = __builtin_bit_cast(dx_bf16x8, make_uint4(ha.x, ha.y, hb.x, hb.y));
  lo = __builtin_bit_cast(dx_bf16x8, make_uint4(la.x, la.y, lb.x, lb.y));
}
__device__ __forceinline__ f32x4 dx_mma_split3(const dx_bf16x8& ah, const dx_bf16x8& al, const dx_bf16x8& bh, const dx_bf16x8& bl, f32x4 c) {
  c = __builtin_amdgcn_mfma_f32_16x16x32_bf16(ah, bl, c, 0, 0, 0);
  c = __builtin_amdgcn_mfma_f32_16x16x32_bf16(al, bh, c, 0, 0, 0);
  c = __builtin_amdgcn_mfma_f32_16x16x32_bf16(ah, bh, c, 0, 0, 0);
  return c;
}

__device__ __forceinline__ float dx_wave_sum(float v) {
#pragma unroll
  for (int off = 32; off > 0; off >>= 1) v += __shfl_xor(v, off, 64);
  return v;
}
__device__ __forceinline__ float dx_wave_max(float v) {
#pragma unroll
  for (int off = 32; off > 0; off >>= 1) v = fmaxf(v, __shfl_xor(v, off, 64));
  return v;
}

__device__ __forceinline__ uint64_t dx_rand64(uint64_t seed, uint64_t idx) {
  uint32_t x = (uint32_t)idx ^ (uint32_t)seed;
  const uint32_t hi = (uint32_t)(idx >> 32) ^ (uint32_t)(seed >> 32);
  x ^= hi * 0x9E3779B1u;
  x ^= x >> 16; x *= 0x7FEB352Du; x ^= x >> 15; x *= 0x846CA68Bu; x ^= x >> 16;
  uint32_t y = (x ^ 0x85EBCA6Bu) * 0xC2B2AE35u; y ^= y >> 15;
  return ((uint64_t)y << 32) | x;
}
__device__ __forceinline__ float dx_dropout_scale(uint64_t seed, uint64_t elem, uint32_t thresh16, float inv_keep) {
  uint64_t r = dx_rand64(seed, elem >> 2);
  uint32_t bits = (uint32_t)(r >> (16 * (elem & 3))) & 0xFFFFu;
  return bits >= thresh16 ? inv_keep : 0.0f;
}
__device__ __forceinline__ float dx_keep_lo(uint32_t w, uint32_t thresh, float x, float alt) {
  float y;
  asm("v_cmp_ge_u16_sdwa vcc, %1, %2 src0_sel:WORD_0 src1_sel:WORD_0\n\tv_cndmask_b32_e32 %0, %4, %3, vcc" : "=v"(y) : "v"(w), "v"(thresh), "v"(x), "v"(alt) : "vcc");
  return y;
}
__device__ __forceinline__ float dx_keep_hi(uint32_t w, uint32_t thresh, float x, float alt) {
  float y;
  asm("v_cmp_ge_u16_sdwa vcc, %1, %2 src0_sel:WORD_1 src1_sel:WORD_0\n\tv_cndmask_b32_e32 %0, %4, %3, vcc" : "=v"(y) : "v"(w), "v"(thresh), "v"(x), "v"(alt) : "vcc");
  return y;
}
__device__ __forceinline__ void dx_keep2(uint32_t bits, uint32_t thresh, float& x, float& y, float alt) {
  asm("v_cmp_ge_u32_e32 vcc, %2, %3\n\tv_cndmask_b32_e32 %0, 0, %0, vcc\n\tv_cndmask_b32_e32 %1, %4, %1, vcc" : "+v"(x), "+v"(y) : "v"(bits), "v"(thresh), "v"(alt) : "vcc");
}
__device__ __forceinline__ void dx_keep4(uint64_t r, uint32_t thresh, float x[4], float alt) {
  const uint32_t lo = (uint32_t)r, hi = (uint32_t)(r >> 32);
  x[0] = dx_keep_lo(lo, thresh, x[0], alt); x[1] = dx_keep_hi(lo, thresh, x[1], alt);
  x[2] = dx_keep_lo(hi, thresh, x[2], alt); x[3] = dx_keep_hi(hi, thresh, x[3], alt);
}
__device__ __forceinline__ void dx_dropout_scale4(uint64_t seed, uint64_t elem0, uint32_t thresh16, float inv_keep, float out[4]) {
  uint64_t r = dx_rand64(seed, elem0 >> 2);
#pragma unroll
  for (int i = 0; i < 4; ++i) out[i] = ((uint32_t)(r >> (16 * i)) & 0xFFFFu) >= thresh16 ? inv_keep : 0.0f;
}
#endif
```

ubisoft_laforge_daft_exprt_amd/csrc/dx_f16_names.h:

```cpp
#pragma once
#define dx_accent_sum dx_accent_sum_f16
#define dx_add_pos dx_add_pos_f16
#define dx_attention_bwd dx_attention_bwd_f16
#define dx_attention_fwd dx_attention_fwd_f16
#define dx_attention_proj_ln_fwd dx_attention_proj_ln_fwd_f16
#define dx_channel_affine dx_channel_affine_f16
#define dx_colsum dx_colsum_f16
#define dx_condition_prosody dx_condition_prosody_f16
#define dx_conv_gemm dx_conv_gemm_f16
#define dx_conv_wgrad dx_conv_wgrad_f16
#define dx_conv_wgrad_batched dx_conv_wgrad_batched_f16
#define dx_cross_entropy dx_cross_entropy_f16
#define dx_embedding_bwd dx_embedding_bwd_f16
#define dx_ff_block_bwd dx_ff_block_bwd_f16
#define dx_ff_pair dx_ff_pair_f16
#define dx_ff_pair_ln dx_ff_pair_ln_f16
#define dx_ff_pair_ln_qkv dx_ff_pair_ln_qkv_f16
#define dx_ff_pair_lnbwd dx_ff_pair_lnbwd_f16
#define dx_gather_speaker_rows dx_gather_speaker_rows_f16
#define dx_l2_normalize dx_l2_normalize_f16
#define dx_length_order dx_length_order_f16
#define dx_ln_bwd dx_ln_bwd_f16
#define dx_film_affine_bwd dx_film_affine_bwd_f16
#define dx_film_affine_fwd dx_film_affine_fwd_f16
#define dx_ln_fwd dx_ln_fwd_f16
#define dx_proj_ln_fwd dx_proj_ln_fwd_f16
#define dx_mask_rows dx_mask_rows_f16
#define dx_mean_pool dx_mean_pool_f16
#define dx_mean_pool_bwd dx_mean_pool_bwd_f16
#define dx_pack_dims dx_pack_dims_f16
#define dx_pitch_chain_bwd dx_pitch_chain_bwd_f16
#define dx_pitch_chain_fwd dx_pitch_chain_fwd_f16
#define dx_pack_weights dx_pack_weights_f16
#define dx_pack_weights_batched dx_pack_weights_batched_f16
#define dx_pack_weights_host dx_pack_weights_host_f16
#define dx_relu_bwd dx_relu_bwd_f16
#define dx_scalar_conv_wgrad dx_scalar_conv_wgrad_f16
#define dx_transpose dx_transpose_f16
#define dx_unpack_wgrad dx_unpack_wgrad_f16
```

ubisoft_laforge_daft_exprt_amd/functional.py:

```python
from __future__ import annotations

import threading

import torch

from . import ops

_seed_state = threading.local()


def manual_seed(seed: int) -> None:
    _seed_state.base = (int(seed) * 0x9E3779B97F4A7C15 + 0x1234567) & 0xFFFFFFFFFFFFFFFF
    _seed_state.counter = 0


def next_seed() -> int:
    if not hasattr(_seed_state, 'base'):
        manual_seed(torch.initial_seed())
    _seed_state.counter += 1
    return (_seed_state.base + _seed_state.counter * 0xD1B54A32D192ED03) & 0xFFFFFFFFFFFFFFFF


def _sink(param, enabled):
    if not enabled or param is None:
        return None
    g = param.grad
    if g is None or not g.is_contiguous() or g.dtype != torch.float32:
        return None
    return g


class Lengths:

    def __init__(self, lengths: torch.Tensor, host=None):
        if not lengths.is_cuda:
            raise RuntimeError('lengths must live on the GPU (the kernels read them as device memory); got a CPU tensor')
        self.host = [int(v) for v in (lengths.tolist() if host is None else host)]
        self.max = max(self.host)
        self.total = sum(self.host)
        self.i32 = lengths.to(dtype=torch.int32).contiguous()
        self.i64 = lengths
        self.exist = None


class LinearFn(torch.autograd.Function):
    @staticmethod
    def forward(ctx, x, weight, bias, pack, relu, grad_scale, lens, need_dx):
        x2 = x.reshape(-1, x.shape[-1]) if lens is None else x
        ctx.prec = pack.rt.precision
        y = ops.conv_gemm(x2, pack, bias, relu=relu, lens=lens, mask_rows=lens is not None, prec=ctx.prec)
        ctx.save_for_backward(x2, y if relu else None)
        ctx.pack, ctx.relu, ctx.grad_scale, ctx.lens, ctx.need_dx, ctx.xshape = pack, relu, grad_scale, lens, need_dx, x.shape
        ctx.params, ctx.sink = (weight, bias), bool(pack.rt.sink)
        return y.view(*x.shape[:-1], y.shape[-1])

    @staticmethod
    def backward(ctx, dy):
        x2, y = ctx.saved_tensors
        dy = dy.contiguous().view(*x2.shape[:-1], dy.shape[-1])
        if ctx.lens is not None:
            dy = ops.mask_rows(dy, ctx.lens)
        if ctx.relu:
            dy = ops.relu_bwd(dy, y)
        dw, db = ops.conv_wgrad(dy, x2, ctx.pack, arena=ctx.pack.rt.arena, w_sink=_sink(ctx.params[0], ctx.sink), b_sink=_sink(ctx.params[1], ctx.sink),
                                prec=ctx.prec, defer=ctx.lens is None)
        dx = None
        if ctx.need_dx:
            dx = ops.conv_gemm(dy, ctx.pack, None, transpose=True, out_scale=ctx.grad_scale, prec=ctx.prec).view(ctx.xshape)
        return dx, dw, db, None, None, None, None, None


class PaddedLinear:

    def __init__(self, weight, bias, rt=None):
        self.weight, self.bias = weight, bias
        self.rt = rt or ops.DEFAULT
        self.cout = weight.shape[0]
        self.cout4 = (self.cout + 3) // 4 * 4
        self._key = None
        self.wpad = self.bpad = self.pack = None

    def padded(self):
        key = (self.weight._version, self.bias._version, self.weight.data_ptr(), self.bias.data_ptr(), self.rt.pack_epoch)
        if key != self._key or (self.wpad is not None and self.wpad.is_cuda and torch.cuda.is_current_stream_capturing()):
            w = self.weight.detach()
            if self.wpad is None or self.wpad.device != w.device:
                self.wpad = torch.zeros(self.cout4, w.shape[1], dtype=w.dtype, device=w.device)
                self.bpad = torch.zeros(self.cout4, dtype=w.dtype, device=w.device)
                self.pack = ops.PackedWeight(self.wpad, self.rt)
            self.wpad[:self.cout].copy_(w)
            self.bpad[:self.cout].copy_(self.bias.detach())
            self._key = key
        return self.wpad, self.bpad, self.pack


class PaddedLinearFn(torch.autograd.Function):
    @staticmethod
    def forward(ctx, x, weight, bias, padded: PaddedLinear):
        _, bpad, pack = padded.padded()
        ctx.prec = pack.rt.precision
        y = ops.conv_gemm(x, pack, bpad, prec=ctx.prec)
        ctx.save_for_backward(x)
        ctx.pack, ctx.cout = pack, padded.cout
        return y[:, :padded.cout].contiguous()

    @staticmethod
    def backward(ctx, dy):
        (x,) = ctx.saved_tensors
        dyp = ops._zeros(ctx.pack.rt.arena, dy.shape[0], ctx.pack.cout, device=dy.device)
        dyp[:, :ctx.cout].copy_(dy)
        dw, db = ops.conv_wgrad(dyp, x, ctx.pack, arena=ctx.pack.rt.arena, prec=ctx.prec)
        dw, db = dw[:ctx.cout], db[:ctx.cout]
        dx = ops.conv_gemm(dyp, ctx.pack, None, transpose=True, prec=ctx.prec)
        return dx, dw, db, None


class FFTBlockFn(torch.autograd.Function):
    @staticmethod
    def forward(ctx, x, film, lens, packs, cfg, training,
                in_w, in_b, out_w, out_b, ln1_w, ln1_b, c1_w, c1_b, c2_w, c2_b, ln2_w, ln2_b, qkv_pre=None, next_in=None):
        p_attn = cfg['attn_dropout'] if training else 0.0
        p_conv = cfg['conv_dropout'] if training else 0.0
        heads = cfg['attn_nb_heads']
        s_attn, s_ln1, s_ln2 = (next_seed(), next_seed(), next_seed()) if training else (0, 0, 0)
        film = film if film is None or film.stride(-1) == 1 else film.contiguous()
        L = lens.i32
        rt = packs['in'].rt
        prec = rt.precision
        hd = ops.hidden_dtype(prec)
        qkv = qkv_pre if qkv_pre is not None else \
            ops.conv_gemm(x, packs['in'], in_b, lens=L, halo=0, out_dtype=hd, prec=prec)
        so = rt.seed_offset
        sh = ops.gemm_shadow(prec)
        if ops.attn_proj_ln_applies(qkv, heads, packs['out'], prec):
            att, lse, z1, y1, mean1, rstd1, *rest = ops.attn_proj_ln_fwd(qkv, lens.i32, heads, s_attn, p_attn, packs['out'], out_b, x, ln1_w, ln1_b, None,
                                                                         seed_pre=s_ln1, p_pre=p_attn, shadow=sh, seed_offset=so, prec=prec)
            y1g = rest[0] if sh else y1
        else:
            att, lse = ops.attention_fwd(qkv, lens.i32, heads, s_attn, p_attn, prec=prec, seed_offset=so, ctx_dtype=hd)
            z1 = ops.conv_gemm(att, packs['out'], out_b, lens=L, halo=0, prec=prec)
            ln1 = ops.ln_fwd(z1, x, ln1_w, ln1_b, None, lens.i32, seed_pre=s_ln1, p_pre=p_attn, shadow=sh, seed_offset=so, prec=prec)
            y1, mean1, rstd1 = ln1[:3]
            y1g = ln1[3] if sh else y1
        fused = ops.ff_pair_applies(y1g, packs['c1'], packs['c2'], prec)
        qkv_next = hmask = None
        if fused:
            if next_in is not None and not ops.next_qkv_applies(next_in[0], prec):
                next_in = None
            need_bwd = any(ctx.needs_input_grad)
            z2, h, y2, mean2, rstd2, *rest = ops.ff_pair_ln(y1g, packs['c1'], packs['c2'], c1_b, c2_b, L, y1, ln2_w, ln2_b, film, seed_pre=s_ln2,
                                                            p_pre=p_conv, seed_offset=so, prec=prec, rows_exist=lens.exist, next_in=next_in,
                                                            need_h=need_bwd,
                                                            want_mask=need_bwd)
            hmask = rest.pop() if need_bwd else None
            qkv_next = rest[0] if rest else None
        else:
            h = ops.conv_gemm(y1g, packs['c1'], c1_b, relu=True, lens=L, halo=1, out_dtype=hd, prec=prec, rows_exist=lens.exist)
            z2 = ops.conv_gemm(h, packs['c2'], c2_b, lens=L, halo=0, prec=prec, rows_exist=lens.exist)
            y2, mean2, rstd2 = ops.ln_fwd(z2, y1, ln2_w, ln2_b, film, lens.i32, seed_pre=s_ln2, p_pre=p_conv, seed_offset=so, prec=prec)
        ctx.save_for_backward(x, film, qkv, att, lse, z1, mean1, rstd1, y1g, h, z2, mean2, rstd2, ln1_w, ln1_b, ln2_w, ln2_b)
        ctx.lens, ctx.packs, ctx.heads = lens, packs, heads
        ctx.drop = (p_attn, p_conv, s_attn, s_ln1, s_ln2)
        ctx.prec, ctx.sink, ctx.fused, ctx.seed_offset = prec, rt.sink, fused, so
        ctx.hmask = hmask
        if qkv_next is not None:
            ctx.mark_non_differentiable(qkv_next)
        ctx.set_materialize_grads(False)
        return y2, qkv_next

    @staticmethod
    def backward(ctx, dy2, _dqkv_next=None):
        x, film, qkv, att, lse, z1, mean1, rstd1, y1, h, z2, mean2, rstd2, ln1_w, ln1_b, ln2_w, ln2_b = ctx.saved_tensors
        lens, packs = ctx.lens, ctx.packs
        E = lens.exist
        p_attn, p_conv, s_attn, s_ln1, s_ln2 = ctx.drop
        dy2 = dy2.contiguous()
        L = lens.i32
        B, _, D = x.shape
        Fc = h.shape[2]
        pad = ops.ZeroArena.padded
        arena = packs['in'].rt.arena or ops.ZeroArena(x.device, 6 * pad(D) + pad(B * 2 * D) + 2 * pad(3 * D * Fc) + pad(Fc) + pad(D * D) + pad(3 * D * D) + pad(3 * D) + 64)
        P = packs.get('params', {})
        prec = ctx.prec
        sk = {k: _sink(v, ctx.sink) for k, v in P.items()}
        g = sk.get
        sh = ops.gemm_shadow(prec)
        so = ctx.seed_offset
        if ctx.fused:
            dz1, dh, dproj, dff, dfilm, dln2_w, dln2_b, dln1_w, dln1_b, datt = ops.ff_block_bwd(
                dy2, z2, mean2, rstd2, ln2_w, ln2_b, film, packs['c1'], packs['c2'], L, h, z1, mean1, rstd1, ln1_w, ln1_b,
                seed2=s_ln2, p2=p_conv, seed1=s_ln1, p1=p_attn, seed_offset=so, prec=prec, arena=arena,
                sinks={'ln2_w': g('ln2_w'), 'ln2_b': g('ln2_b'), 'ln1_w': g('ln1_w'), 'ln1_b': g('ln1_b')},
                out_pack=packs['out'], hmask=ctx.hmask, rows_exist=E)
            dc2_w, dc2_b = ops.conv_wgrad(dff, h, packs['c2'], L, 0, arena=arena, w_sink=g('c2_w'), b_sink=g('c2_b'), prec=prec, defer=True, rows_exist=E)
        else:
            datt = None
            r2 = ops.ln_bwd(dy2, z2, mean2, rstd2, ln2_w, ln2_b, film, L, want_da=p_conv > 0, seed_pre=s_ln2, seed_offset=so, prec=prec,
                            p_pre=p_conv, arena=arena, w_sink=g('ln2_w'), b_sink=g('ln2_b'), shadow=sh)
            dz2, da2, dln2_w, dln2_b, dfilm = r2[:5]
            dff = r2[5] if sh else (da2 if da2 is not None else dz2)
            dc2_w, dc2_b = ops.conv_wgrad(dff, h, packs['c2'], L, 0, arena=arena, w_sink=g('c2_w'), b_sink=g('c2_b'), prec=prec, defer=True, rows_exist=E)
            dh = ops.conv_gemm(dff, packs['c2'], None, transpose=True, relu_aux=h, lens=L, halo=1, out_dtype=h.dtype, prec=prec, rows_exist=E)
            dy1 = ops.conv_gemm(dh, packs['c1'], None, transpose=True, out=dz2, accumulate=True, lens=L, halo=0, prec=prec,
                                rows_exist=E)
            r1 = ops.ln_bwd(dy1, z1, mean1, rstd1, ln1_w, ln1_b, None, L, want_da=p_attn > 0, seed_pre=s_ln1, seed_offset=so, prec=prec,
                            p_pre=p_attn, arena=arena, w_sink=g('ln1_w'), b_sink=g('ln1_b'), shadow=sh)
            dz1, da1, dln1_w, dln1_b = r1[:4]
            dproj = r1[5] if sh else (da1 if da1 is not None else dz1)
        dc1_w, dc1_b = ops.conv_wgrad(dh, y1, packs['c1'], L, 1, arena=arena, w_sink=g('c1_w'), b_sink=g('c1_b'), prec=prec, defer=True, rows_exist=E)
        dout_w, dout_b = ops.conv_wgrad(dproj, att, packs['out'], L, 0, arena=arena, w_sink=g('out_w'), b_sink=g('out_b'), prec=prec, defer=True)
        if datt is None:
            datt = ops.conv_gemm(dproj, packs['out'], None, transpose=True, lens=L, halo=0, prec=prec, out_dtype=att.dtype)
        dqkv = ops.attention_bwd(qkv, att, datt, lse, L, ctx.heads, s_attn, p_attn, out_dtype=qkv.dtype, prec=prec, seed_offset=so)
        din_w, din_b = ops.conv_wgrad(dqkv, x, packs['in'], L, 0, arena=arena, w_sink=g('in_w'), b_sink=g('in_b'), prec=prec, defer=True)
        dx = ops.conv_gemm(dqkv, packs['in'], None, transpose=True, out=dz1, accumulate=True, lens=L, halo=0, prec=prec)
        return (dx, dfilm, None, None, None, None,
                din_w, din_b, dout_w, dout_b, dln1_w, dln1_b, dc1_w, dc1_b, dc2_w, dc2_b, dln2_w, dln2_b, None, None)


def cut(rt, level, t):
    sp = None if rt is None else rt.backward_split
    if sp is None or level > rt.cut_levels or not t.requires_grad:
        return t
    leaf = t.detach().requires_grad_(True)
    sp.append((level, t, leaf))
    return leaf


class AccentFront0Fn(torch.autograd.Function):
    @staticmethod
    def forward(ctx, mel, lens, packs, p_drop, training, c0_w, c0_b, l0_w, l0_b):
        p = p_drop if training else 0.0
        seed = next_seed() if training else 0
        x0 = ops.transpose(mel.contiguous())
        L = lens.i32
        rt = packs['p0'].rt
        prec = rt.precision
        hd = ops.hidden_dtype(prec)
        so = rt.seed_offset
        h0 = ops.conv_gemm(x0, packs['p0'], c0_b, relu=True, lens=L, halo=2, out_dtype=hd, prec=prec, rows_exist=lens.exist)
        y0, m0, r0 = ops.ln_fwd(h0, None, l0_w, l0_b, None, L, seed_post=seed, p_post=p, halo=2, seed_offset=so, prec=prec)
        ctx.save_for_backward(x0, h0, m0, r0, l0_w, l0_b)
        ctx.lens, ctx.packs, ctx.p, ctx.seed = lens, packs, p, seed
        ctx.prec, ctx.sink, ctx.seed_offset = prec, rt.sink, so
        return y0

    @staticmethod
    def backward(ctx, dy0):
        x0, h0, m0, r0, l0_w, l0_b = ctx.saved_tensors
        lens, packs, p = ctx.lens, ctx.packs, ctx.p
        arena = packs['p0'].rt.arena
        L = lens.i32
        sk = {k: _sink(v, ctx.sink) for k, v in packs.get('params', {}).items()}
        g = sk.get
        dz0, _, dl0_w, dl0_b, _ = ops.ln_bwd(dy0.contiguous(), h0, m0, r0, l0_w, l0_b, None, L, relu_mask=True, seed_post=ctx.seed, p_post=p,
                                              seed_offset=ctx.seed_offset, prec=ctx.prec, w_sink=g('l0_w'), b_sink=g('l0_b'), halo=2, arena=arena)
        dc0_w, dc0_b = ops.conv_wgrad(dz0, x0, packs['p0'], L, 2, w_sink=g('c0_w'), b_sink=g('c0_b'), prec=ctx.prec, arena=arena, rows_exist=lens.exist)
        return None, None, None, None, None, dc0_w, dc0_b, dl0_w, dl0_b


class AccentFront12Fn(torch.autograd.Function):
    @staticmethod
    def forward(ctx, y0, energy, pitch, lens, packs, pe, p_drop, training,
                c1_w, c1_b, l1_w, l1_b, c2_w, c2_b, l2_w, l2_b, we, be, wp, bp):
        p = p_drop if training else 0.0
        seeds = [next_seed() if training else 0 for _ in range(2)]
        L = lens.i32
        rt = packs['p1'].rt
        prec = rt.precision
        hd = ops.hidden_dtype(prec)
        so = rt.seed_offset
        h1 = ops.conv_gemm(y0, packs['p1'], c1_b, relu=True, lens=L, halo=1, out_dtype=hd, prec=prec, rows_exist=lens.exist)
        y1, m1, r1 = ops.ln_fwd(h1, None, l1_w, l1_b, None, L, seed_post=seeds[0], p_post=p, halo=1, seed_offset=so, prec=prec)
        h2 = ops.conv_gemm(y1, packs['p2'], c2_b, relu=True, lens=L, halo=0, prec=prec, rows_exist=lens.exist)
        y2, m2, r2 = ops.ln_fwd(h2, None, l2_w, l2_b, None, L, seed_post=seeds[1], p_post=p, halo=0, seed_offset=so, prec=prec)
        energy, pitch = energy.contiguous(), pitch.contiguous()
        out = ops.accent_sum(y2, energy, pitch, we, be, wp, bp, pe, lens.i32)
        ctx.save_for_backward(y0, h1, m1, r1, y1, h2, m2, r2, energy, pitch, l1_w, l1_b, l2_w, l2_b)
        ctx.lens, ctx.packs, ctx.p, ctx.seeds = lens, packs, p, seeds
        ctx.emb_params = (we, be, wp, bp)
        ctx.prec, ctx.sink, ctx.seed_offset = prec, rt.sink, so
        return out

    @staticmethod
    def backward(ctx, dout):
        y0, h1, m1, r1, y1, h2, m2, r2, energy, pitch, l1_w, l1_b, l2_w, l2_b = ctx.saved_tensors
        lens, packs, p, seeds = ctx.lens, ctx.packs, ctx.p, ctx.seeds
        so = ctx.seed_offset
        arena = packs['p1'].rt.arena
        dout = ops.mask_rows(dout.contiguous(), lens.i32)
        dwe, dbe, dwp, dbp = ops.scalar_conv_wgrad(dout, energy, pitch, lens.i32, sinks=tuple(_sink(q, ctx.sink) for q in ctx.emb_params))
        L = lens.i32
        prec = ctx.prec
        sk = {k: _sink(v, ctx.sink) for k, v in packs.get('params', {}).items()}
        g = sk.get
        dz2, _, dl2_w, dl2_b, _ = ops.ln_bwd(dout, h2, m2, r2, l2_w, l2_b, None, L, relu_mask=True, seed_post=seeds[1], p_post=p, seed_offset=so, prec=prec,
                                              w_sink=g('l2_w'), b_sink=g('l2_b'), halo=0, arena=arena)
        E = lens.exist
        dc2_w, dc2_b = ops.conv_wgrad(dz2, y1, packs['p2'], L, 0, w_sink=g('c2_w'), b_sink=g('c2_b'), prec=prec, arena=arena, rows_exist=E)
        dy1 = ops.conv_gemm(dz2, packs['p2'], None, transpose=True, lens=L, halo=1, out_dtype=h1.dtype, prec=prec, rows_exist=E)
        dz1, _, dl1_w, dl1_b, _ = ops.ln_bwd(dy1, h1, m1, r1, l1_w, l1_b, None, L, relu_mask=True, seed_post=seeds[0], p_post=p, seed_offset=so, prec=prec,
                                              w_sink=g('l1_w'), b_sink=g('l1_b'), halo=1, arena=arena)
        dc1_w, dc1_b = ops.conv_wgrad(dz1, y0, packs['p1'], L, 1, w_sink=g('c1_w'), b_sink=g('c1_b'), prec=prec, arena=arena, rows_exist=E)
        dy0 = ops.conv_gemm(dz1, packs['p1'], None, transpose=True, lens=L, halo=2, out_dtype=y0.dtype, prec=prec, rows_exist=E)
        return (dy0, None, None, None, None, None, None, None,
                dc1_w, dc1_b, dl1_w, dl1_b, dc2_w, dc2_b, dl2_w, dl2_b, dwe, dbe, dwp, dbp)


class SplitFilmFn(torch.autograd.Function):

    @staticmethod
    def forward(ctx, film):
        ctx.shape = film.shape
        t = film.transpose(0, 1).contiguous()
        return tuple(t[i] for i in range(film.shape[1]))

    @staticmethod
    def backward(ctx, *grads):
        B, nb, C2 = ctx.shape
        ref = next(g for g in grads if g is not None)
        return torch.stack([g if g is not None else torch.zeros_like(ref) for g in grads], dim=1)


class FilmAffineFn(torch.autograd.Function):

    @staticmethod
    def forward(ctx, gammas, betas, pm, nb, rt):
        gammas, betas = gammas.contiguous(), betas.contiguous()
        pmc = None if pm is None else pm.detach().contiguous()
        film = ops.film_affine_fwd(gammas, betas, pmc, nb)
        ctx.save_for_backward(gammas, betas, pmc)
        ctx.nb, ctx.rt, ctx.has_pm = nb, rt, pm is not None
        whole = film.detach()
        ctx.mark_non_differentiable(whole)
        ctx.set_materialize_grads(False)
        return tuple(film[i] for i in range(nb)) + (whole,)

    @staticmethod
    def backward(ctx, *grads):
        gammas, betas, pm = ctx.saved_tensors
        dg, db, dpm = ops.film_affine_bwd(list(grads[:ctx.nb]), gammas, betas, pm, arena=None if ctx.rt is None else ctx.rt.arena)
        return dg, db, dpm, None, None


class MeanPoolFn(torch.autograd.Function):

    @staticmethod
    def forward(ctx, x, lens, rt=None):
        ctx.lens, ctx.N = lens, x.shape[1]
        return ops.mean_pool(x, lens.i32, arena=None if rt is None else rt.arena)

    @staticmethod
    def backward(ctx, dout):
        return ops.mean_pool_bwd(dout.contiguous(), ctx.lens.i32, ctx.N), None, None


class EmbedPosFn(torch.autograd.Function):

    @staticmethod
    def forward(ctx, symbols, emb, pe, lens, rt=None):
        symbols = symbols.contiguous()
        ctx.save_for_backward(symbols)
        ctx.lens, ctx.rows, ctx.rt = lens, emb.shape[0], rt
        ctx.emb, ctx.sink = emb, bool(rt is not None and rt.sink)
        return ops.add_pos(None, symbols, emb, pe, lens.i32)

# ... 72 lines not shown
```

ubisoft_laforge_daft_exprt_amd/ops.py:

```python
from __future__ import annotations

import ctypes

import torch

from . import _lib
from ._lib import lib

PRECISIONS = ('f32', 'bf16', 'fp16', 'bf16x3')


class Runtime:

    def __init__(self, precision='f32'):
        self.precision = _check_precision(precision)
        self.pack_epoch = 0
        self.sink = False
        self.launch_log = None
        self.arena = None
        self.arena_hint = 1 << 20
        self.seed_offset = None
        self.defer_wgrad = False
        self.wgrad_queue = {}
        self.backward_split = None
# ... 302 lines not shown
                                  _p(z), _p(mean), _p(rstd), _p(ln_w), _p(ln_b), _p(dg), _p(dw), _p(db), seed_pre, float(p_pre), _p(seed_offset), _stream())
    return out, dh, dg, (None if w_sink is not None else dw), (None if b_sink is not None else db)


def ff_block_bwd(dy2, z2, mean2, rstd2, ln2_w, ln2_b, film, pack1: PackedWeight, pack2: PackedWeight, lens, aux, z1, mean1, rstd1, ln1_w, ln1_b, *,
                 seed2=0, p2=0.0, seed1=0, p1=0.0, seed_offset=None, halo=1, prec=None, arena=None, sinks=None, out_pack=None, hmask=None,
                 rows_exist=None):
    prec = pack1.rt.precision if prec is None else prec
    B, N, D = dy2.shape
    Fc = pack1.cout
    dev = dy2.device
    sinks = sinks or {}
    i1, i2 = pack1.image(prec), pack2.image(prec)
    dz1 = torch.empty(B, N, 128, dtype=torch.float32, device=dev)
    dh = torch.empty(B, N, Fc, dtype=_H16[prec], device=dev)
    dg1 = torch.empty(B, N, 128, dtype=_H16[prec], device=dev)
    dg2 = torch.empty(B, N, 128, dtype=_H16[prec], device=dev)
    acc = {k: (sinks.get(k) if sinks.get(k) is not None else _zeros(arena, 128, device=dev)) for k in ('ln2_w', 'ln2_b', 'ln1_w', 'ln1_b')}
    dfilm = _zeros(arena, B, 256, device=dev) if film is not None else None
    datt = wt = None
    if out_pack is not None:
        if out_pack.cin != 128 or out_pack.cout != 128 or out_pack.taps != 1:
            raise ValueError('out_pack must be the (128, 128) out-projection')
        wt = out_pack.image(prec).bwd
        datt = torch.empty(B, N, 128, dtype=_H16[prec], device=dev)
    _log(pack1, ('ffpair', B * N, N, 128, Fc, 3))
    _fn('dx_ff_block_bwd', prec)(_p(dy2), _p(z2), _p(mean2), _p(rstd2), _p(ln2_w), _p(ln2_b), _p(film), 0 if film is None else film.stride(0),
                                 _p(dg2), _p(acc['ln2_w']), _p(acc['ln2_b']), _p(dfilm), 256, seed2, float(p2),
                                 _p(i2.bwd), _p(i1.bwd), _p(aux), _rows(aux), _p(dh), _rows(dh), _p(dz1), B, N, Fc, _p(lens), int(halo),
                                 _p(z1), _p(mean1), _p(rstd1), _p(ln1_w), _p(ln1_b), _p(dg1), _p(acc['ln1_w']), _p(acc['ln1_b']),
                                 seed1, float(p1), _p(wt), _p(datt), _p(seed_offset), _p(hmask), _p(rows_exist), _stream())
    ret = lambda k: None if sinks.get(k) is not None else acc[k]
    return dz1, dh, dg1, dg2, dfilm, ret('ln2_w'), ret('ln2_b'), ret('ln1_w'), ret('ln1_b'), datt


class ZeroArena:

    def __init__(self, device, n_floats):
        self.buf = torch.zeros(int(n_floats), dtype=torch.float32, device=device)
        self.off = 0
        self.requested = 0

    @staticmethod
    def padded(n):
        return (int(n) + 3) // 4 * 4

    def take(self, *shape):
        n = 1
        for d in shape:
            n *= int(d)
        self.requested += self.padded(n)
        if self.off + n > self.buf.numel():
            return torch.zeros(*shape, dtype=torch.float32, device=self.buf.device)
        out = torch.empty(0, dtype=torch.float32, device=self.buf.device).set_(self.buf.untyped_storage(), self.off, tuple(int(d) for d in shape))
        self.off += self.padded(n)
        return out


def begin_step_arena(rt: Runtime, device) -> None:
    rt.arena = ZeroArena(device, rt.arena_hint)


def end_step_arena(rt: Runtime) -> None:
    if rt.arena is not None:
        rt.arena_hint = max(rt.arena_hint, int(1.25 * rt.arena.requested))
        rt.arena = None


def _zeros(arena, *shape, device=None):
    return arena.take(*shape) if arena is not None else torch.zeros(*shape, dtype=torch.float32, device=device)


def conv_wgrad(dy, x, pack: PackedWeight, lens=None, halo=-1, bias=True, arena=None, w_sink=None, b_sink=None, prec=None, defer=False,
               rows_exist=None):
    B_, N_ = (1, x.shape[0]) if x.dim() == 2 else (x.shape[0], x.shape[1])
    g = w_sink if w_sink is not None else _zeros(arena, *pack.weight.shape, device=x.device)
    db = b_sink if b_sink is not None else (_zeros(arena, pack.cout, device=x.device) if bias else None)
    _log(pack, ('wgrad', B_ * N_, N_, pack.cin, pack.cout, pack.taps))
    prec = prec or pack.rt.precision
    _check_h16(prec, dy, x)
    rt = pack.rt
    if (defer and rt.defer_wgrad and w_sink is not None and (b_sink is not None or not bias) and _half(prec) and pack.cin % 128 == 0
            and pack.cout % 8 == 0 and _rows(dy) % 8 == 0 and _rows(x) % 8 == 0):
        key = (pack.taps, _is_bf16(dy), _is_bf16(x), prec)
        rt.wgrad_queue.setdefault(key, []).append(((_p(dy), _p(x), _p(g), _p(db), _p(lens), _rows(dy), _rows(x), B_, N_, pack.cin, pack.cout,
                                                    int(halo), 0, _p(rows_exist)), (dy, x, g, db, lens, rows_exist)))
        return None, None
    _fn('dx_conv_wgrad', prec)(_p(dy), _rows(dy), _p(x), _rows(x), _p(g), B_, N_, pack.cin, pack.cout, pack.taps, _p(lens), int(halo),
                               _mode(prec), _is_bf16(dy), _is_bf16(x), _p(db), _p(rows_exist), _stream())
    return (None if w_sink is not None else g), (None if b_sink is not None else db)


class _WgradJob(ctypes.Structure):
    _fields_ = [(n, ctypes.c_void_p) for n in ('dY', 'X', 'G', 'dbias', 'lens')] + \
               [(n, ctypes.c_int) for n in ('ldy', 'ldx', 'B', 'N', 'Cin', 'Cout', 'skip_halo', 'reserved')] + \
               [('rows_exist', ctypes.c_void_p)]


WGRAD_BATCH = {1: 32, 3: 8}
WGRAD_BATCH_LOG = {}


def flush_wgrads(rt) -> int:
    launches = 0
    for (taps, dyh, xh, prec), jobs in rt.wgrad_queue.items():
        jobs.sort(key=lambda j: -j[0][7] * j[0][8])
        for i in range(0, len(jobs), WGRAD_BATCH[taps]):
            part = jobs[i:i + WGRAD_BATCH[taps]]
            arr = (_WgradJob * len(part))(*[_WgradJob(*fields) for fields, _ in part])
            if _lib.TIMER is not None:
                WGRAD_BATCH_LOG[ctypes.addressof(arr)] = (arr, [fields for fields, _ in part])
            _fn('dx_conv_wgrad_batched', prec)(ctypes.addressof(arr), len(part), taps, dyh, xh, _stream())
            launches += 1
    rt.wgrad_queue.clear()
    return launches


def film_affine_fwd(gammas, betas, pm, nb):
    B, total = gammas.shape
    C = total // nb
    film = torch.empty(nb, B, 2 * C, dtype=torch.float32, device=gammas.device)
    lib().dx_film_affine_fwd(_p(gammas), _p(betas), _p(pm), _p(film), B, nb, C, _stream())
    return film


def film_affine_bwd(dfilms, gammas, betas, pm, arena=None):
    B, total = gammas.shape
    nb = len(dfilms)
    C = total // nb
    dfilms = [None if g is None else g.contiguous() for g in dfilms]
    ptrs = (ctypes.c_void_p * nb)(*[None if g is None else g.data_ptr() for g in dfilms])
    dg, db = torch.empty_like(gammas), torch.empty_like(betas)
    dpm = _zeros(arena, 2, nb, device=gammas.device) if pm is not None else None
    lib().dx_film_affine_bwd(ctypes.addressof(ptrs), _p(gammas), _p(betas), _p(pm), _p(dg), _p(db), _p(dpm), B, nb, C, _stream())
    return dg, db, dpm


def colsum(x, C=None):
    C = x.shape[-1] if C is None else C
    rows = x.numel() // x.shape[-1]
    out = torch.zeros(C, dtype=torch.float32, device=x.device)
    lib().dx_colsum(_p(x), _rows(x), _p(out), rows, C, _is_bf16(x), _stream())
    return out




def length_order(lens_i32):
    order = torch.empty_like(lens_i32)
    lib().dx_length_order(_p(lens_i32), _p(order), lens_i32.shape[0], _stream())
    return order


def attention_fwd(qkv, lens, heads, seed, p_drop, prec=None, seed_offset=None, ctx_dtype=torch.float32, order=None):
    B, N, D3 = qkv.shape
    D = D3 // 3
    ctx = torch.empty(B, N, D, dtype=ctx_dtype, device=qkv.device)
    lse = torch.empty(B, heads, N, dtype=torch.float32, device=qkv.device)
    prec = prec or DEFAULT.precision
    _check_h16(prec, qkv, ctx)
    _fn('dx_attention_fwd', prec)(_p(qkv), _rows(qkv), _p(lens), _p(ctx), D, _p(lse), B, N, heads, D, seed, _p(seed_offset), float(p_drop),
                           _mode(prec), _is_bf16(qkv), _is_bf16(ctx), _p(order), _stream())
    return ctx, lse


def attention_bwd(qkv, ctx, dctx, lse, lens, heads, seed, p_drop, out_dtype=torch.float32, prec=None, seed_offset=None, order=None):
    B, N, D3 = qkv.shape
    D = D3 // 3
    if dctx.dtype != ctx.dtype:
        raise TypeError(f'ctx ({ctx.dtype}) and dctx ({dctx.dtype}) must be stored alike')
    dqkv = torch.empty(B, N, D3, dtype=out_dtype, device=qkv.device)
    delta = torch.empty(B, heads, N, dtype=torch.float32, device=qkv.device)
    prec = prec or DEFAULT.precision
    _fn('dx_attention_bwd', prec)(_p(qkv), _rows(qkv), _p(ctx), _p(dctx), _rows(dctx), _p(lse), _p(delta), _p(lens), _p(dqkv), _rows(dqkv),
                           B, N, heads, D, seed, _p(seed_offset), float(p_drop), _mode(prec), _is_bf16(qkv), _is_bf16(dqkv), _is_bf16(ctx),
                           _p(order), _stream())
    return dqkv


def gemm_shadow(prec=None):
    return bool(_half(prec or DEFAULT.precision))


def ln_fwd(a, res, w, b, film, lens, *, seed_pre=0, p_pre=0.0, seed_post=0, p_post=0.0, halo=0, shadow=False, seed_offset=None, prec=None):
    B, N, C = a.shape
    y = torch.empty_like(a)
    prec = prec or DEFAULT.precision
    y_h = torch.empty(B, N, C, dtype=_H16[prec], device=a.device) if shadow else None
    mean = torch.empty(B, N, dtype=torch.float32, device=a.device)
    rstd = torch.empty(B, N, dtype=torch.float32, device=a.device)
    _fn('dx_ln_fwd', prec)(_p(a), _p(res), _p(w), _p(b), _p(film), 0 if film is None else film.stride(0), _p(lens), int(halo), _p(y), _p(mean), _p(rstd),
                    B, N, C, seed_pre, float(p_pre), seed_post, float(p_post), _p(seed_offset), _is_bf16(a), _p(y_h), _stream())
    return (y, mean, rstd, y_h) if shadow else (y, mean, rstd)


def attn_proj_ln_applies(qkv, heads, pack: PackedWeight, prec) -> bool:
    return (prec in _H16 and qkv.dtype == _H16[prec] and qkv.dim() == 3 and qkv.shape[2] == 384 and heads == 2
            and pack.taps == 1 and pack.cin == 128 and pack.cout == 128)


def attn_proj_ln_fwd(qkv, lens, heads, seed, p_drop, pack: PackedWeight, proj_bias, res, w, b, film, *, seed_pre=0, p_pre=0.0, shadow=False,
                     seed_offset=None, prec=None):
    B, N, D3 = qkv.shape
    D = D3 // 3
    prec = prec or pack.rt.precision
    _check_h16(prec, qkv)
    h16 = _H16[prec]
    ctx = torch.empty(B, N, D, dtype=h16, device=qkv.device)
    lse = torch.empty(B, heads, N, dtype=torch.float32, device=qkv.device)
    z = torch.empty(B, N, D, dtype=torch.float32, device=qkv.device)
    y = torch.empty_like(z)
    y_h = torch.empty(B, N, D, dtype=h16, device=qkv.device) if shadow else None
    mean = torch.empty(B, N, dtype=torch.float32, device=qkv.device)
    rstd = torch.empty(B, N, dtype=torch.float32, device=qkv.device)
    img = pack.image(prec)
    _log(pack, ('gemm', B * N, N, pack.cin, pack.cout, 1))
    _fn('dx_attention_proj_ln_fwd', prec)(_p(qkv), _rows(qkv), _p(lens), _p(ctx), D, _p(lse), B, N, heads, D, seed, _p(seed_offset), float(p_drop),
                                          _p(img.fwd), _p(proj_bias), _p(z), _p(res), _p(w), _p(b), _p(film), 0 if film is None else film.stride(0),
                                          _p(y), _p(mean), _p(rstd), seed_pre, float(p_pre), _p(y_h), _stream())
    return (ctx, lse, z, y, mean, rstd, y_h) if shadow else (ctx, lse, z, y, mean, rstd)


def proj_ln_fwd(x, pack: PackedWeight, proj_bias, res, w, b, film, lens, *, seed_pre=0, p_pre=0.0, halo=0, shadow=False, seed_offset=None, prec=None):
    B, N, C = x.shape
    prec = prec or pack.rt.precision
    _check_h16(prec, x)
    img = pack.image(prec)
    z = torch.empty(B, N, C, dtype=torch.float32, device=x.device)
    y = torch.empty_like(z)
    y_h = torch.empty(B, N, C, dtype=_H16[prec], device=x.device) if shadow else None
    mean = torch.empty(B, N, dtype=torch.float32, device=x.device)
    rstd = torch.empty(B, N, dtype=torch.float32, device=x.device)
    _log(pack, ('gemm', B * N, N, pack.cin, pack.cout, 1))
    _fn('dx_proj_ln_fwd', prec)(_p(x), _rows(x), _p(img.fwd), _p(proj_bias), _p(z), _p(res), _p(w), _p(b), _p(film), 0 if film is None else film.stride(0),
                                _p(lens), int(halo), _p(y), _p(mean), _p(rstd), B, N, seed_pre, float(p_pre), _p(seed_offset), _p(y_h), _stream())
    return (z, y, mean, rstd, y_h) if shadow else (z, y, mean, rstd)


def ln_bwd(dy, z, mean, rstd, w, b, film, lens, *, relu_mask=False, want_da=False, seed_pre=0, p_pre=0.0, seed_post=0, p_post=0.0,
           arena=None, w_sink=None, b_sink=None, halo=0, shadow=False, seed_offset=None, prec=None):
    B, N, C = z.shape
    dz = torch.empty_like(z)
    prec = prec or DEFAULT.precision
    dg_h = torch.empty(B, N, C, dtype=_H16[prec], device=z.device) if shadow else None
    da = torch.empty_like(z) if (want_da and not shadow) else None
    dw = w_sink if w_sink is not None else _zeros(arena, C, device=z.device)
    db = b_sink if b_sink is not None else _zeros(arena, C, device=z.device)
    dfilm = _zeros(arena, B, 2 * C, device=z.device) if film is not None else None
    _fn('dx_ln_bwd', prec)(_p(dy), _p(z), _p(mean), _p(rstd), _p(w), _p(b), _p(film), 0 if film is None else film.stride(0), _p(lens), int(halo),
                    _p(dz), _p(da), _p(dw), _p(db), _p(dfilm), 2 * C, B, N, C, int(relu_mask),
                    seed_pre, float(p_pre), seed_post, float(p_post), _p(seed_offset), _is_bf16(z), _p(dg_h), _stream())
    out = (dz, da, (None if w_sink is not None else dw), (None if b_sink is not None else db), dfilm)
    return out + (dg_h,) if shadow else out


def add_pos(x, sym, emb, pe, lens):
    if emb is not None:
        B, N = sym.shape
        D = emb.shape[1]
    else:
        B, N, D = x.shape
    out = torch.empty(B, N, D, dtype=torch.float32, device=pe.device)
    lib().dx_add_pos(_p(x), _p(sym), _p(emb), _p(pe), _p(lens), _p(out), B, N, D, pe.shape[0], _stream())
    return out


def mask_rows(x, lens):
    B, N, C = x.shape
    out = torch.empty_like(x)
    lib().dx_mask_rows(_p(x), _p(lens), _p(out), B, N, C, _stream())
    return out


def embedding_bwd(dout, sym, lens, n_rows, arena=None, sink=None):
    B, N, D = dout.shape
    demb = sink if sink is not None else _zeros(arena, n_rows, D, device=dout.device)
    lib().dx_embedding_bwd(_p(dout), _p(sym), _p(lens), _p(demb), B, N, D, _stream())
    return None if sink is not None else demb


def accent_sum(prenet, energy, pitch, we, be, wp, bp, pe, lens):
    B, N, D = prenet.shape
    out = torch.empty_like(prenet)
    lib().dx_accent_sum(_p(prenet), _p(energy), _p(pitch), _p(we), _p(be), _p(wp), _p(bp), _p(pe), _p(lens), _p(out), B, N, D, pe.shape[0], _stream())
    return out


def scalar_conv_wgrad(dout, s0, s1, lens, rowscale=None, sinks=None):
    B, N = s0.shape
    D = 128
    dev = s0.device
    sinks = sinks or (None, None, None, None)
    dw0 = sinks[0] if sinks[0] is not None else torch.zeros(D, 1, 3, dtype=torch.float32, device=dev)
    db0 = sinks[1] if sinks[1] is not None else torch.zeros(D, dtype=torch.float32, device=dev)
    dw1 = (sinks[2] if sinks[2] is not None else torch.zeros(D, 1, 3, dtype=torch.float32, device=dev)) if s1 is not None else None
    db1 = (sinks[3] if sinks[3] is not None else torch.zeros(D, dtype=torch.float32, device=dev)) if s1 is not None else None
    ldd = dout.stride(-2) if dout.dim() == 3 else 0
    lib().dx_scalar_conv_wgrad(_p(dout), ldd, _p(rowscale), _p(s0), _p(s1), _p(lens), _p(dw0), _p(db0), _p(dw1), _p(db1), B, N, D, _stream())
    return tuple(None if sk is not None else t for sk, t in zip(sinks, (dw0, db0, dw1, db1)))


def mean_pool(x, lens, arena=None):
    B, N, C = x.shape
    out = _zeros(arena, B, C, device=x.device)
    lib().dx_mean_pool(_p(x), _p(lens), _p(out), B, N, C, _stream())
    return out


def mean_pool_bwd(dout, lens, N):
    B, C = dout.shape
    dx = torch.empty(B, N, C, dtype=torch.float32, device=dout.device)
    lib().dx_mean_pool_bwd(_p(dout), _p(lens), _p(dx), B, N, C, _stream())
    return dx


def transpose(x, add_to=None):
    B, R, C = x.shape
    out = add_to if add_to is not None else torch.empty(B, C, R, dtype=torch.float32, device=x.device)
    lib().dx_transpose(_p(x), _p(out), B, R, C, int(add_to is not None), _stream())
    return out


def l2_normalize(x):
    y = torch.empty_like(x)
    lib().dx_l2_normalize(_p(x), _p(y), x.shape[0], x.shape[1], _stream())
    return y


def cross_entropy(logits, target):
    B, S = logits.shape
    loss = torch.empty(1, dtype=torch.float32, device=logits.device)
    dlogits = torch.empty_like(logits)
    lib().dx_cross_entropy(_p(logits), _p(target), _p(loss), _p(dlogits), B, S, _stream())
    return loss, dlogits


def duration_scan(dur_int):
    B, L = dur_int.shape
    mu = torch.empty(B, L, dtype=torch.float32, device=dur_int.device)
    totals = torch.empty(B, dtype=torch.long, device=dur_int.device)
    lib().dx_duration_scan(_p(dur_int), _p(mu), _p(totals), B, L, _stream())
    return mu, totals


def upsample_prep(enc, dur, energy, pitch, wd, bd, we, be, wp, bp, wr, br, lens):
    B, L, D = enc.shape
    xs = torch.empty_like(enc)
    z = torch.empty(B, L, dtype=torch.float32, device=enc.device)
    sigma = torch.empty(B, L, dtype=torch.float32, device=enc.device)
    lib().dx_upsample_prep(_p(enc), _p(dur), _p(energy), _p(pitch), _p(wd), _p(bd), _p(we), _p(be), _p(wp), _p(bp), _p(wr), _p(br),
                           _p(lens), _p(xs), _p(z), _p(sigma), B, L, D, _stream())
    return xs, z, sigma


def upsample_fwd(xs, mu, sigma, lens, T):
    B, L, D = xs.shape
    weights = torch.empty(B, L, T, dtype=torch.float32, device=xs.device)
    xup = torch.empty(B, T, D, dtype=torch.float32, device=xs.device)
    lib().dx_upsample_fwd(_p(xs), _p(mu), _p(sigma), _p(lens), _p(weights), _p(xup), B, L, T, D, _stream())
    return xup, weights


def upsample_bwd(dxup, xs, mu, sigma, weights, lens, arena=None):
    B, L, D = xs.shape
    T = weights.shape[2]
    dxs = _zeros(arena, B, L, D, device=xs.device)
    dsigma = _zeros(arena, B, L, device=xs.device)
    lib().dx_upsample_bwd(_p(dxup), _p(xs), _p(mu), _p(sigma), _p(weights), _p(lens), _p(dxs), _p(dsigma), B, L, T, D, _stream())
    return dxs, dsigma


def upsample_sym_bwd(dxs, dsigma, xs, z, dur, lens, wd, bd, wr, dwr_sink=None, dbr_sink=None):
# ... 110 lines not shown
```

ubisoft_laforge_daft_exprt_amd/profiling.py:

```python
from __future__ import annotations

from collections import OrderedDict

PEAK_TFLOPS = {'f32': 157.3, 'bf16': 2500.0, 'bf16x3': 2500.0 / 3}
PEAK_HBM_GBS = 8000.0


class Geometry:

    def __init__(self, axes):
        self.by_n = {}
        for lens in axes:
            lens = [int(v) for v in lens]
            self.by_n[(len(lens), max(lens))] = (sum(lens), sum(v * v for v in lens))

    def rows(self, B, N, lens_ptr=True):
        if not lens_ptr:
            return B * N
        return self.by_n.get((B, N), (B * N, B * N * N))[0]

    def pairs(self, B, N):
        return self.by_n.get((B, N), (B * N, B * N * N))[1]


def _conv_route(a):
    if not a['bf16']:
        return 'conv_gemm_kernel<f32>'
    if a['bf16'] == 2:
        return 'conv_gemm_kernel<bf16x3>'
    cinp = (a['Cin'] + 63) // 64 * 64
    if cinp >= 256 and a['Cin'] % 64 == 0:
        return f"conv_dk_kernel<{a['taps']}>"
    if cinp == 128 and a['B'] * ((a['N'] + 127) // 128) >= 64:
        return f"conv_ws_kernel<{a['taps']}>"
    return 'conv_gemm_kernel<bf16>'


def price(name, a, geom: Geometry):
    g = a.get
    has = lambda k: bool(g(k))
    if name.endswith('_f16'):
        name = name[:-4]
    if name == 'dx_conv_gemm':
        rows = geom.rows(a['B'], a['N'], has('lens'))
        xb, yb, ab = (2 if a['x_bf16'] else 4), (2 if a['y_bf16'] else 4), (2 if a['aux_bf16'] else 4)
        wb = 2 if a['bf16'] == 1 else 4
        byt = rows * (a['Cin'] * xb + a['Cout'] * yb * (2 if a['accumulate'] else 1) + (a['Cout'] * ab if has('relu_aux') else 0)) \
            + a['taps'] * a['Cin'] * a['Cout'] * wb
        return _conv_route(a), 'mfma', 2.0 * a['taps'] * a['Cin'] * a['Cout'] * rows, byt
    if name == 'dx_ff_pair':
        rows = geom.rows(a['B'], a['N'], has('lens'))
        F = a['F']
        byt = rows * (128 * 2 + F * 2 + 128 * 4 * (2 if a['accumulate'] else 1) + (F * 2 if has('aux') else 0)) + 2 * 3 * 128 * F * 2
        return 'ff_pair_kernel<bwd>' if has('aux') else 'ff_pair_kernel<fwd>', 'mfma', 2.0 * 2 * 3 * 128 * F * rows, byt
    if name == 'dx_ff_pair_ln':
        rows = geom.rows(a['B'], a['N'], has('lens'))
        F = a['F']
        byt = rows * (128 * 2 + F * 2 + 128 * 4 * 3 + 8) + 2 * 3 * 128 * F * 2
        return 'ff_pair_kernel<fwd>', 'mfma', 2.0 * 2 * 3 * 128 * F * rows, byt
    if name == 'dx_ff_pair_ln_qkv':
        rows = geom.rows(a['B'], a['N'], has('lens'))
        F = a['F']
        byt = rows * (128 * 2 + F * 2 + 128 * 4 * 3 + 8 + 384 * 2) + 2 * 3 * 128 * F * 2 + 384 * 128 * 2
        return 'ff_pair_kernel<fwd>', 'mfma', (2.0 * 2 * 3 * 128 * F + 2.0 * 128 * 384) * rows, byt
    if name == 'dx_ff_pair_lnbwd':
        rows = geom.rows(a['B'], a['N'], has('lens'))
        F = a['F']
        byt = rows * (128 * 2 + 2 * F * 2 + 128 * 4 * 3 + 128 * 2 + 8) + 2 * 3 * 128 * F * 2
        return 'ff_pair_kernel<bwd>', 'mfma', 2.0 * 2 * 3 * 128 * F * rows, byt
    if name == 'dx_ff_block_bwd':
        rows = geom.rows(a['B'], a['N'], has('lens'))
        F = a['F']
        byt = rows * (2 * 128 * 4 + 2 * 128 * 4 + 2 * 128 * 2 + 2 * F * 2 + 128 * 4 + 16) + 2 * 3 * 128 * F * 2
        return 'ff_pair_kernel<bwd>', 'mfma', 2.0 * 2 * 3 * 128 * F * rows, byt
    if name == 'dx_conv_wgrad':
        rows = geom.rows(a['B'], a['N'], has('lens'))
        byt = rows * (a['Cout'] * (2 if a['dy_bf16'] else 4) + a['Cin'] * (2 if a['x_bf16'] else 4)) + a['taps'] * a['Cin'] * a['Cout'] * 4
        wide = a['Cin'] % 128 == 0 and -(-a['Cout'] // 128) * -(-a['Cin'] // 64) >= 64
        label = (f"wgrad_split_kernel<{a['taps']},bf16x3>" if a['bf16'] == 2
                 else f"wgrad_bf16_kernel<{a['taps']}{',wide' if wide else ''}>" if a['bf16'] and a['Cin'] % 8 == 0 and a['Cout'] % 8 == 0
                 else f"wgrad_kernel<{a['taps']}>")
        return label, 'mfma', 2.0 * a['taps'] * a['Cin'] * a['Cout'] * rows, byt
    if name == 'dx_conv_wgrad_batched':
        from . import ops
        jobs = ops.WGRAD_BATCH_LOG.get(a['jobs'], (None, []))[1]
        flops = byt = 0
        for (_dy, _x, _g, _db, lens, _ldy, _ldx, B, N, Cin, Cout, *_rest) in jobs:
            rows = geom.rows(B, N, lens is not None)
            flops += 2.0 * a['taps'] * Cin * Cout * rows
            byt += rows * (Cout * (2 if a['dy_bf16'] else 4) + Cin * (2 if a['x_bf16'] else 4)) + a['taps'] * Cin * Cout * 4
        return f"wgrad_bf16_kernel<{a['taps']},wide>", 'mfma', (flops or None), (byt or None)
    if name in ('dx_attention_fwd', 'dx_attention_bwd'):
        rows, pairs = geom.rows(a['B'], a['N']), geom.pairs(a['B'], a['N'])
        D, H = a['D'], a['H']
        qb = 2 if a['qkv_bf16'] else 4
        sfx = ' <bf16x3>' if a['bf16'] == 2 else ''
        if name == 'dx_attention_fwd':
            return 'attn_fwd' + sfx, 'mfma', 4.0 * pairs * D, rows * (3 * D * qb + D * 4 + H * 4)
        gb = 2 if a['dqkv_bf16'] else 4
        return 'attn_bwd (dq + dkv)' + sfx, 'mfma', 14.0 * pairs * D, rows * (2 * 3 * D * qb + 2 * D * 4 + 3 * D * gb + 2 * H * 4)
    if name in ('dx_pitch_chain_fwd', 'dx_pitch_chain_bwd'):
        rows = geom.rows(a['B'], a['T'], True)
        flops = 2.0 * 3 * (a['M'] * 256 + 2 * 256 * 256 + 256) * rows
        byt = rows * (a['M'] * 4 + 4 + 96 + (a['M'] * 8 if name.endswith('bwd') else 0))
        return ('pitch_chain<fwd>' if name.endswith('fwd') else 'pitch_chain<bwd>'), 'mfma', flops, byt
    if name == 'dx_attention_proj_ln_fwd':
        rows, pairs = geom.rows(a['B'], a['N']), geom.pairs(a['B'], a['N'])
        D, H = a['D'], a['H']
        byt = rows * (3 * D * 2 + D * 2 + H * 4) + rows * (128 * (4 + 4 + (4 if has('res') else 0) + (2 if has('y_bf16_copy') else 0)) + 8) + 128 * 128 * 2
        return 'attn_fwd+proj_ln', 'mfma', 4.0 * pairs * D + 2.0 * rows * 128 * 128, byt
    if name == 'dx_ln_fwd':
        rows = geom.rows(a['B'], a['N'], has('lens'))
        C, ab = a['C'], (2 if a['io_bf16'] else 4)
        byt = rows * (C * (2 * ab + 4 + (4 if has('res') else 0) + (2 if has('y_bf16_copy') else 0)) + 8)
        return f'ln_fwd_kernel<{C}>', 'hbm', None, byt
    if name == 'dx_proj_ln_fwd':
        rows = geom.rows(a['B'], a['N'], has('lens'))
        byt = rows * (128 * (2 + 4 + 4 + (4 if has('res') else 0) + (2 if has('y_bf16_copy') else 0)) + 8) + 128 * 128 * 2
        return 'proj_ln_fwd', 'hbm', None, byt
    if name == 'dx_ln_bwd':
        rows = geom.rows(a['B'], a['N'], has('lens'))
        C, zb = a['C'], (2 if a['io_bf16'] else 4)
        byt = rows * (C * (3 * zb + (4 if has('da') else 0) + (2 if has('dg_bf16_copy') else 0)) + 8)
        return f'ln_bwd_kernel<{C}>', 'hbm', None, byt
    if name == 'dx_upsample_fwd':
        B, L, T, D = a['B'], a['L'], a['T'], a['D']
        return 'upsample_fwd', 'hbm', None, B * L * D * 4 + 3 * B * L * 4 + B * T * D * 4 + B * L * T * 4
    if name == 'dx_upsample_bwd':
        B, L, T, D = a['B'], a['L'], a['T'], a['D']
        return 'upsample_bwd (dsigma + dxs)', 'hbm', None, B * T * D * 4 + B * L * T * 4 + 2 * B * L * D * 4 + 3 * B * L * 4
    if name in ('dx_upsample_prep', 'dx_upsample_sym_bwd'):
        return name[3:], 'hbm', None, 2 * a['B'] * a['L'] * a['D'] * 4 + 6 * a['B'] * a['L'] * 4
    if name == 'dx_adam_step':
        return 'adam_kernel', 'hbm', None, a['n'] * 28
    if name == 'dx_sumsq':
        return 'sumsq_kernel', 'hbm', None, a['n'] * 4
    if name == 'dx_mel_stats':
        return 'mel_stats', 'hbm', None, 2 * a['B'] * a['M'] * a['T'] * 4
    if name == 'dx_mel_grad':
        return 'mel_grad', 'hbm', None, 3 * a['B'] * a['M'] * a['T'] * 4
    if name == 'dx_add_pos':
        rows = geom.rows(a['B'], a['N'])
        return 'add_pos', 'hbm', None, rows * a['D'] * 4 * (2 if has('x') else 1)
    if name == 'dx_accent_sum':
        return 'accent_sum', 'hbm', None, geom.rows(a['B'], a['N']) * (2 * a['D'] * 4 + 8)
    if name == 'dx_scalar_conv_wgrad':
        return 'scalar_conv_wgrad', 'hbm', None, geom.rows(a['B'], a['N']) * (a['D'] * 4 if a['ldd'] else 0) + geom.rows(a['B'], a['N']) * 8
    if name == 'dx_transpose':
        return 'transpose', 'hbm', None, 2 * a['B'] * a['R'] * a['Cc'] * 4
    if name == 'dx_mask_rows':
        return 'mask_rows', 'hbm', None, 2 * geom.rows(a['B'], a['N']) * a['C'] * 4
    if name == 'dx_mean_pool':
        return 'mean_pool', 'hbm', None, geom.rows(a['B'], a['N']) * a['C'] * 4
    if name == 'dx_mean_pool_bwd':
        return 'mean_pool_bwd', 'hbm', None, geom.rows(a['B'], a['N']) * a['C'] * 4
    if name == 'dx_channel_affine':
        return 'channel_affine', 'hbm', None, 2 * a['rows'] * a['C'] * (2 if a.get('io_bf16') else 4)
    if name == 'dx_relu_bwd':
        return 'relu_bwd', 'hbm', None, 3 * a['n'] * 4
    if name == 'dx_colsum':
        return 'colsum', 'hbm', None, a['rows'] * a['C'] * (2 if a['x_bf16'] else 4)
    return name[3:], 'hbm', None, None


def summarize(records, geom: Geometry, precision: str):
    rows = {}
    for name, args, ev0, ev1 in records:
        label, bound, flops, byt = price(name, args, geom)
        e = rows.setdefault(label, {'launches': 0, 'total_us': 0.0, 'bound': bound, 'flops': 0.0, 'bytes': 0.0, 'unpriced': 0})
        e['launches'] += 1
        e['total_us'] += ev0.elapsed_time(ev1) * 1e3
        if bound == 'mfma' and flops is not None:
            e['flops'] += flops
        if byt is not None:
            e['bytes'] += byt
        else:
            e['unpriced'] += 1
    out = OrderedDict()
    for label, e in sorted(rows.items(), key=lambda kv: -kv[1]['total_us']):
        t = e['total_us'] * 1e-6
        r = {'launches': e['launches'], 'total_us': round(e['total_us'], 1), 'avg_us': round(e['total_us'] / e['launches'], 2), 'bound': e['bound']}
        if e['bound'] == 'mfma':
            peak = PEAK_TFLOPS['bf16x3' if 'bf16x3>' in label else 'f32' if '<f32>' in label or precision in ('f32', 'bf16x3') else 'bf16']
            r.update(achieved=round(e['flops'] / t / 1e12, 2), unit='TFLOP/s', peak=peak, frac=round(e['flops'] / t / 1e12 / peak, 4),
                     algorithmic_bytes_per_launch=int(e['bytes'] / e['launches']))
        elif e['unpriced'] == 0:
            r.update(achieved=round(e['bytes'] / t / 1e9, 1), unit='GB/s', peak=PEAK_HBM_GBS, frac=round(e['bytes'] / t / 1e9 / PEAK_HBM_GBS, 4),
                     algorithmic_bytes_per_launch=int(e['bytes'] / e['launches']))
        out[label] = r
    return out
```

Baseline: 4.877 million.

## Record attention dropout keep bits in forward and replay them in backward

The forward attention kernels now write a bitmask of dropout keep decisions per 64x64 tile into a global buffer. The backward dq and dkv kernels read that mask instead of regenerating the random numbers with the hash. This trades the hash arithmetic in both backward kernels for extra global writes in forward and reads in backward, plus a B*H*T*T*256 int16 buffer held between passes. It applies only in half-precision training with attention dropout enabled.

```diff
diff --git a/include/daft_exprt_hip.h b/include/daft_exprt_hip.h
--- a/include/daft_exprt_hip.h
+++ b/include/daft_exprt_hip.h
@@ -71,6 +71,17 @@
 int dx_attention_bwd(const void* qkv, int ld, const void* ctx, const void* dctx, int ldc, const float* lse, float* delta,
                      const int* lens, void* dqkv, int ldg, int B, int N, int H, int D, uint64_t seed, const uint64_t* seed_offset, float p_drop, int bf16,
                      int qkv_bf16, int dqkv_bf16, int ctx_bf16, const int* order, void* stream);
+int dx_attention_fwd_keep(const void* qkv, int ld, const int* lens, void* ctx, int ldc, float* lse,
+                          int B, int N, int H, int D, uint64_t seed, const uint64_t* seed_offset, float p_drop, int bf16, int qkv_bf16, int ctx_bf16,
+                          const int* order, void* keep, void* stream);
+int dx_attention_proj_ln_fwd_keep(const void* qkv, int ld, const int* lens, void* ctx, int ldc, float* lse, int B, int N, int H, int D,
+                                  uint64_t seed, const uint64_t* seed_offset, float p_drop,
+                                  const void* Wpack, const float* proj_bias, float* z, const float* res, const float* w, const float* bias,
+                                  const float* film, int ld_film, float* y, float* mean, float* rstd, uint64_t seed_pre, float p_pre,
+                                  void* y_bf16_copy, void* keep, void* stream);
+int dx_attention_bwd_keep(const void* qkv, int ld, const void* ctx, const void* dctx, int ldc, const float* lse, float* delta,
+                          const int* lens, void* dqkv, int ldg, int B, int N, int H, int D, uint64_t seed, const uint64_t* seed_offset, float p_drop,
+                          int bf16, int qkv_bf16, int dqkv_bf16, int ctx_bf16, const int* order, const void* keep, void* stream);
 
 int dx_ln_fwd(void* a, const void* res, const float* w, const float* bias, const float* film, int ld_film,
               const int* lens, int halo, void* y, float* mean, float* rstd, int B, int N, int C,
diff --git a/ubisoft_laforge_daft_exprt_amd/csrc/dx_attention.hip b/ubisoft_laforge_daft_exprt_amd/csrc/dx_attention.hip
--- a/ubisoft_laforge_daft_exprt_amd/csrc/dx_attention.hip
+++ b/ubisoft_laforge_daft_exprt_amd/csrc/dx_attention.hip
@@ -21,6 +21,7 @@
   const uint64_t* seed_offset;
   const int* order;
   int xcd_map;
+  uint16_t* keep;
 };
 
 __device__ __forceinline__ f32x4 mma4(const float4& a, const float4& b, f32x4 c) {
@@ -189,6 +190,7 @@
   const uint64_t* seed_offset;
   const int* order;
   int xcd_map;
+  const uint16_t* keep;
 };
 
 __global__ __launch_bounds__(256, 2) void attn_bwd_dq_kernel(const AttnBwdArgs a_) {
@@ -774,6 +776,15 @@
 #define DX_MFMA_BF16(A, B, C) DX_MFMA_H16((A), (B), (C))
 __device__ __forceinline__ float dx_max2(float a, float b) { return __builtin_amdgcn_fmed3f(a, b, INFINITY); }
 
+__device__ __forceinline__ size_t keep_block(int bh, int T, int qt, int kt) { return (((size_t)bh * T + qt) * T + kt) * 256; }
+
+__device__ __forceinline__ uint32_t keep_valid_mask(int kbase, int g, int len) {
+  uint32_t m = 0;
+#pragma unroll
+  for (int i = 0; i < 16; ++i) m = 2 * m + (kbase + (i >> 2) * 16 + g * 4 + (i & 3) < len ? 1u : 0u);
+  return m;
+}
+
 template <typename QT, typename CT>
 __global__ __launch_bounds__(256, 2) void attn_fwd_bf16_kernel(const AttnArgs a_) {
   AttnArgs a = a_;
@@ -808,6 +819,7 @@
   const int ntiles = (len + 63) / 64;
   const uint64_t drow = (uint64_t)((size_t)bh * a.N + qrow) << 14;
   const uint32_t thresh_v = a.thresh;
+  uint16_t* const kp = a.keep ? a.keep + keep_block(bh, (a.N + 63) >> 6, blk.tile, 0) + wave * 64 + lane : nullptr;
   f32x4 kreg[4], vreg[4];
   DX_TILE_LOAD(QT, kreg, base, a.ld, a.D + h * HD, 0, a.N)
   DX_TILE_LOAD(QT, vreg, base, a.ld, 2 * a.D + h * HD, 0, a.N)
@@ -842,6 +854,7 @@
     const float m_new = dx_max2(m_run, mx);
     const bool rescale = __builtin_amdgcn_ballot_w64(m_new > m_run) != 0;
     float ls = 0.f;
+    uint32_t kbits = 0;
 #pragma unroll
     for (int kt = 0; kt < 4; ++kt) {
       float pk[4];
@@ -850,12 +863,16 @@
         pk[e] = __builtin_amdgcn_exp2f(st[kt][e] - m_new);
         ls += pk[e];
       }
-      if (a.thresh) dx_keep4(dx_rand64(a.seed, drow | (uint64_t)((kbase + kt * 16 + g * 4) >> 2)), thresh_v, pk, 0.f);
+      if (a.thresh) dx_keep4_rec(dx_rand64(a.seed, drow | (uint64_t)((kbase + kt * 16 + g * 4) >> 2)), thresh_v, pk, 0.f, kbits);
 #pragma unroll
       for (int e = 0; e < 4; ++e) st[kt][e] = pk[e];
     }
     ls += __shfl_xor(ls, 16, 64);
     ls += __shfl_xor(ls, 32, 64);
+    if (kp) {
+      if (tail_tile) kbits &= keep_valid_mask(kbase, g, len);
+      kp[(size_t)kt0 * 256] = qrow < len ? (uint16_t)kbits : (uint16_t)0;
+    }
     if (rescale) {
       const float alpha = __builtin_amdgcn_exp2f(m_run - m_new);
       l_run *= alpha;
@@ -955,6 +972,7 @@
   const int ntiles = (len + 63) / 64;
   const uint64_t drow = (uint64_t)((size_t)bh * a.N + qrow) << 14;
   const uint32_t thresh_v = a.thresh;
+  uint16_t* const kp = a.keep ? a.keep + keep_block(bh, ntx, q0 >> 6, 0) + wq * 64 + lane : nullptr;
   f32x4 kreg[4], vreg[4];
   DX_TILE_LOAD(QT, kreg, base, a.ld, a.D + h * HD, 0, a.N)
   DX_TILE_LOAD(QT, vreg, base, a.ld, 2 * a.D + h * HD, 0, a.N)
@@ -989,6 +1007,7 @@
     const float m_new = dx_max2(m_run, mx);
     const bool rescale = __builtin_amdgcn_ballot_w64(m_new > m_run) != 0;
     float ls = 0.f;
+    uint32_t kbits = 0;
 #pragma unroll
     for (int kt = 0; kt < 4; ++kt) {
       float pk[4];
@@ -997,12 +1016,16 @@
         pk[e] = __builtin_amdgcn_exp2f(st[kt][e] - m_new);
         ls += pk[e];
       }
-      if (a.thresh) dx_keep4(dx_rand64(a.seed, drow | (uint64_t)((kbase + kt * 16 + g * 4) >> 2)), thresh_v, pk, 0.f);
+      if (a.thresh) dx_keep4_rec(dx_rand64(a.seed, drow | (uint64_t)((kbase + kt * 16 + g * 4) >> 2)), thresh_v, pk, 0.f, kbits);
 #pragma unroll
       for (int e = 0; e < 4; ++e) st[kt][e] = pk[e];
     }
     ls += __shfl_xor(ls, 16, 64);
     ls += __shfl_xor(ls, 32, 64);
+    if (kp) {
+      if (tail_tile) kbits &= keep_valid_mask(kbase, g, len);
+      kp[(size_t)kt0 * 256] = qrow < len ? (uint16_t)kbits : (uint16_t)0;
+    }
     if (rescale) {
       const float alpha = __builtin_amdgcn_exp2f(m_run - m_new);
       l_run *= alpha;
@@ -1135,7 +1158,7 @@
   for (int e = 0; e < 8; ++e) v[e] = (float)h[e];
 }
 
-template <typename QT, typename OT, typename CT>
+template <typename QT, typename OT, typename CT, bool KEEP>
 __global__ __launch_bounds__(256, 2) void attn_bwd_dq_bf16_kernel(const AttnBwdArgs a_) {
   AttnBwdArgs a = a_;
   if (a.seed_offset) a.seed += *a.seed_offset;
@@ -1186,6 +1209,8 @@
   const int ntiles = (len + 63) / 64;
   const uint64_t drow = (uint64_t)((size_t)bh * a.N + qrow) << 14;
   const uint32_t thresh_v = a.thresh;
+  const uint16_t* const kp = KEEP ? a.keep + keep_block(bh, (a.N + 63) >> 6, blk.tile, 0) + wave * 64 + lane : nullptr;
+  uint32_t knext = KEEP ? kp[0] : 0u;
   f32x4 kreg[4], vreg[4];
   DX_TILE_LOAD(QT, kreg, base, a.ld, a.D + h * HD, 0, a.N)
   DX_TILE_LOAD(QT, vreg, base, a.ld, 2 * a.D + h * HD, 0, a.N)
@@ -1195,9 +1220,11 @@
     DX_TILE_STORE(QT, kreg, Ks)
     DX_TILE_STORE(QT, vreg, Vs)
     __syncthreads();
+    uint32_t kbits = knext << 16;
     if (kt0 + 1 < ntiles) {
       DX_TILE_LOAD(QT, kreg, base, a.ld, a.D + h * HD, kbase + 64, a.N)
       DX_TILE_LOAD(QT, vreg, base, a.ld, 2 * a.D + h * HD, kbase + 64, a.N)
+      if constexpr (KEEP) knext = kp[(size_t)(kt0 + 1) * 256];
     }
     f32x4 ds[4];
     const bool tail_tile = kbase + 64 > len;
@@ -1210,7 +1237,8 @@
         dp = DX_MFMA_BF16(row_frag(Vs, kt * 16 + r, ks, g), gf[ks], dp);
       }
       float u[4] = {dp[0] - delta_q, dp[1] - delta_q, dp[2] - delta_q, dp[3] - delta_q};
-      if (a.thresh) dx_keep4(dx_rand64(a.seed, drow | (uint64_t)((kbase + kt * 16 + g * 4) >> 2)), thresh_v, u, neg_delta_q);
+      if constexpr (KEEP) dx_keep4_replay(kbits, u, neg_delta_q);
+      else if (a.thresh) dx_keep4(dx_rand64(a.seed, drow | (uint64_t)((kbase + kt * 16 + g * 4) >> 2)), thresh_v, u, neg_delta_q);
       float p[4];
 #pragma unroll
       for (int e = 0; e < 4; ++e) p[e] = __builtin_amdgcn_exp2f(s[e]);
@@ -1240,7 +1268,7 @@
   }
 }
 
-template <typename QT, typename OT, typename CT>
+template <typename QT, typename OT, typename CT, bool KEEP>
 __global__ __launch_bounds__(256, (sizeof(QT) == 2 && sizeof(CT) == 2) ? 3 : 2) void attn_bwd_dkv_bf16_kernel(const AttnBwdArgs a_) {
   AttnBwdArgs a = a_;
   if (a.seed_offset) a.seed += *a.seed_offset;
@@ -1278,6 +1306,9 @@
   }
   const uint32_t fsel = 0x0c0c0000u | (uint32_t)((2 * (krow & 3) + 1) << 8) | (uint32_t)(2 * (krow & 3));
   const uint32_t thresh_v = a.thresh;
+  const int T = (a.N + 63) >> 6;
+  const uint16_t* const kp = KEEP ? a.keep + keep_block(bh, T, 0, blk.tile) + 16 * (r >> 2) + 4 * g : nullptr;
+  const int kshift = 4 * wave + (r & 3);
   f32x4 dk[4], dv[4];
 #pragma unroll
   for (int dt = 0; dt < 4; ++dt) { dk[dt] = f32x4{0.f, 0.f, 0.f, 0.f}; dv[dt] = f32x4{0.f, 0.f, 0.f, 0.f}; }
@@ -1289,6 +1320,11 @@
   if (tid < 64 && tid < a.N) { lse_r = a.lse[(size_t)bh * a.N + tid]; delta_r = a.delta[(size_t)bh * a.N + tid]; }
   for (int qt0 = 0; qt0 < ntiles; ++qt0) {
     const int qbase = qt0 * 64;
+    uint2 kw[4];
+    if constexpr (KEEP) {
+#pragma unroll
+      for (int qt = 0; qt < 4; ++qt) kw[qt] = *reinterpret_cast<const uint2*>(kp + ((size_t)qt0 * T * 4 + qt) * 64);
+    }
     __syncthreads();
     DX_TILE_STORE(QT, qreg, Qs)
     DX_TILE_STORE(CT, greg, Gs)
@@ -1309,7 +1345,7 @@
       for (int q2 = 0; q2 < 2; ++q2) {
         const int qt = half * 2 + q2;
         uint32_t wlo = 0, whi = 0;
-        if (a.thresh) {
+        if (!KEEP && a.thresh) {
           const uint64_t w = dx_rand64(a.seed, drop_index(bh, a.N, qbase + qt * 16 + g * 4 + (r & 3), krow) >> 2);
           wlo = (uint32_t)w; whi = (uint32_t)(w >> 32);
         }
@@ -1330,7 +1366,13 @@
         float pk[4] = {p[0], p[1], p[2], p[3]}, u[4], nd[4];
 #pragma unroll
         for (int e = 0; e < 4; ++e) { nd[e] = -delta_s[qt * 16 + g * 4 + e]; u[e] = dp[e] + nd[e]; }
-        if (a.thresh) {
+        if constexpr (KEEP) {
+          const uint32_t w0 = kw[qt].x << kshift, w1 = kw[qt].y << kshift;
+          dx_keep2_bit15<0>(w0, pk[0], u[0], nd[0]);
+          dx_keep2_bit15<1>(w0, pk[1], u[1], nd[1]);
+          dx_keep2_bit15<0>(w1, pk[2], u[2], nd[2]);
+          dx_keep2_bit15<1>(w1, pk[3], u[3], nd[3]);
+        } else if (a.thresh) {
           const uint32_t lo0 = __builtin_amdgcn_mov_dpp(wlo, 0x00, 0xF, 0xF, true), hi0 = __builtin_amdgcn_mov_dpp(whi, 0x00, 0xF, 0xF, true);
           const uint32_t lo1 = __builtin_amdgcn_mov_dpp(wlo, 0x55, 0xF, 0xF, true), hi1 = __builtin_amdgcn_mov_dpp(whi, 0x55, 0xF, 0xF, true);
           const uint32_t lo2 = __builtin_amdgcn_mov_dpp(wlo, 0xAA, 0xF, 0xF, true), hi2 = __builtin_amdgcn_mov_dpp(whi, 0xAA, 0xF, 0xF, true);
@@ -1391,6 +1433,14 @@
 
 extern "C" {
 
+int dx_attention_fwd_keep(const void*, int, const int*, void*, int, float*, int, int, int, int, uint64_t, const uint64_t*, float, int, int, int,
+                          const int*, void*, void*);
+int dx_attention_proj_ln_fwd_keep(const void*, int, const int*, void*, int, float*, int, int, int, int, uint64_t, const uint64_t*, float,
+                                  const void*, const float*, float*, const float*, const float*, const float*, const float*, int, float*, float*,
+                                  float*, uint64_t, float, void*, void*, void*);
+int dx_attention_bwd_keep(const void*, int, const void*, const void*, int, const float*, float*, const int*, void*, int, int, int, int, int,
+                          uint64_t, const uint64_t*, float, int, int, int, int, const int*, const void*, void*);
+
 int dx_length_order(const int* lens, int* order, int B, void* stream) {
   DX_REQUIRE(lens && order && B > 0 && B <= 1024, "dx_length_order: bad arguments (B <= 1024)");
   hipLaunchKernelGGL(length_order_kernel, dim3(1), dim3(1024), 0, (hipStream_t)stream, lens, order, B);
@@ -1401,6 +1451,12 @@
 int dx_attention_fwd(const void* qkvv, int ld, const int* lens, void* ctxv, int ldc, float* lse,
                      int B, int N, int H, int D, uint64_t seed, const uint64_t* seed_offset, float p_drop, int bf16, int qkv_bf16, int ctx_bf16,
                      const int* order, void* stream) {
+  return dx_attention_fwd_keep(qkvv, ld, lens, ctxv, ldc, lse, B, N, H, D, seed, seed_offset, p_drop, bf16, qkv_bf16, ctx_bf16, order, nullptr, stream);
+}
+
+int dx_attention_fwd_keep(const void* qkvv, int ld, const int* lens, void* ctxv, int ldc, float* lse,
+                          int B, int N, int H, int D, uint64_t seed, const uint64_t* seed_offset, float p_drop, int bf16, int qkv_bf16, int ctx_bf16,
+                          const int* order, void* keep, void* stream) {
   float* ctx = (float*)ctxv;
   const float* qkv = (const float*)qkvv;
   if (int rc = check_common("dx_attention_fwd", qkv, ld, B, N, H, D)) return rc;
@@ -1411,8 +1467,10 @@
   DX_REQUIRE(lens && ctx && lse && ldc >= D && (ldc % 4) == 0 && ((uintptr_t)ctx % 16) == 0, "dx_attention_fwd: bad output arguments");
   DX_REQUIRE(!ctx_bf16 || (bf16 && (ldc % 8) == 0), "dx_attention_fwd: a 16-bit context needs the 16-bit operand mode and ldc %% 8 == 0");
   DX_REQUIRE(p_drop >= 0.f && p_drop < 1.f, "dx_attention_fwd: dropout p out of range");
+  DX_REQUIRE(!keep || (bf16 && ((uintptr_t)keep % 16) == 0), "dx_attention_fwd: keep bits need the 16-bit operand mode and 16-byte alignment");
   AttnArgs a{qkv, ld, lens, ctx, ldc, lse, B, N, H, D, seed, (uint32_t)lrintf(p_drop * 65536.f), 1.f / (1.f - p_drop), seed_offset, order, 0};
   a.xcd_map = (H * B) % 8 == 0;
+  a.keep = a.thresh ? (uint16_t*)keep : nullptr;
   hipStream_t s = (hipStream_t)stream;
   dx_prof_begin(DX_PROF_ATTN_FWD, s);
   const dim3 grid(dx_cdiv(N, 64), H, B);
@@ -1432,6 +1490,15 @@
                              const void* Wpack, const float* proj_bias, float* z, const float* res, const float* w, const float* bias,
                              const float* film, int ld_film, float* y, float* mean, float* rstd, uint64_t seed_pre, float p_pre,
                              void* y_bf16_copy, void* stream) {
+  return dx_attention_proj_ln_fwd_keep(qkv, ld, lens, ctx, ldc, lse, B, N, H, D, seed, seed_offset, p_drop, Wpack, proj_bias, z, res, w, bias,
+                                       film, ld_film, y, mean, rstd, seed_pre, p_pre, y_bf16_copy, nullptr, stream);
+}
+
+int dx_attention_proj_ln_fwd_keep(const void* qkv, int ld, const int* lens, void* ctx, int ldc, float* lse, int B, int N, int H, int D,
+                                  uint64_t seed, const uint64_t* seed_offset, float p_drop,
+                                  const void* Wpack, const float* proj_bias, float* z, const float* res, const float* w, const float* bias,
+                                  const float* film, int ld_film, float* y, float* mean, float* rstd, uint64_t seed_pre, float p_pre,
+                                  void* y_bf16_copy, void* keep, void* stream) {
   if (int rc = check_common("dx_attention_proj_ln_fwd", qkv, ld, B, N, H, D)) return rc;
   DX_REQUIRE(H == 2 && D == 128 && (ld % 8) == 0 && (ldc % 8) == 0 && ldc >= D, "dx_attention_proj_ln_fwd: 2 heads x 64, 16-bit rows (ld, ldc multiples of 8)");
   DX_REQUIRE(lens && ctx && lse && Wpack && z && w && bias && y && mean && rstd, "dx_attention_proj_ln_fwd: null pointer");
@@ -1439,11 +1506,13 @@
              (!res || ((uintptr_t)res % 16) == 0), "dx_attention_proj_ln_fwd: pointers must be 16-byte aligned");
   DX_REQUIRE(p_drop >= 0.f && p_drop < 1.f && p_pre >= 0.f && p_pre < 1.f, "dx_attention_proj_ln_fwd: dropout p out of range");
   DX_REQUIRE(!film || ld_film >= 256, "dx_attention_proj_ln_fwd: ld_film too small");
+  DX_REQUIRE(((uintptr_t)keep % 16) == 0, "dx_attention_proj_ln_fwd: keep bits must be 16-byte aligned");
   AttnProjLnArgs k{};
   k.at = AttnArgs{(const float*)qkv, ld, lens, (float*)ctx, ldc, lse, B, N, H, D, seed, (uint32_t)lrintf(p_drop * 65536.f), 1.f / (1.f - p_drop), seed_offset, nullptr, 0};
   k.Wp = (const dx_h16*)Wpack; k.proj_bias = proj_bias; k.z = z; k.res = res; k.w = w; k.bias = bias; k.film = film; k.ld_film = ld_film;
   k.y = y; k.y_h = (dx_h16*)y_bf16_copy; k.mean = mean; k.rstd = rstd;
   k.seed_pre = seed_pre; k.thresh_pre = (uint32_t)lrintf(p_pre * 65536.f); k.inv_keep_pre = 1.f / (1.f - p_pre);
+  k.at.keep = k.at.thresh ? (uint16_t*)keep : nullptr;
   hipStream_t s = (hipStream_t)stream;
   dx_prof_begin(DX_PROF_ATTN_FWD, s);
   hipLaunchKernelGGL(attn_proj_ln_fwd_kernel, dim3(8 * dx_cdiv(N, 64) * dx_cdiv(B, 8)), dim3(512), 0, s, k);
@@ -1455,6 +1524,13 @@
 int dx_attention_bwd(const void* qkvv, int ld, const void* ctxv, const void* dctxv, int ldc, const float* lse, float* delta,
                      const int* lens, void* dqkvv, int ldg, int B, int N, int H, int D, uint64_t seed, const uint64_t* seed_offset, float p_drop, int bf16,
                      int qkv_bf16, int dqkv_bf16, int ctx_bf16, const int* order, void* stream) {
+  return dx_attention_bwd_keep(qkvv, ld, ctxv, dctxv, ldc, lse, delta, lens, dqkvv, ldg, B, N, H, D, seed, seed_offset, p_drop, bf16,
+                               qkv_bf16, dqkv_bf16, ctx_bf16, order, nullptr, stream);
+}
+
+int dx_attention_bwd_keep(const void* qkvv, int ld, const void* ctxv, const void* dctxv, int ldc, const float* lse, float* delta,
+                          const int* lens, void* dqkvv, int ldg, int B, int N, int H, int D, uint64_t seed, const uint64_t* seed_offset, float p_drop,
+                          int bf16, int qkv_bf16, int dqkv_bf16, int ctx_bf16, const int* order, const void* keep, void* stream) {
   const float* qkv = (const float*)qkvv; float* dqkv = (float*)dqkvv; const float* ctx = (const float*)ctxv; const float* dctx = (const float*)dctxv;
   DX_REQUIRE(bf16 == 0 || bf16 == 1 || (bf16 == 2 && kSplitBuild), "dx_attention_bwd: bad operand mode %d", bf16);
   const bool split = bf16 == 2;
@@ -1466,28 +1542,31 @@
   DX_REQUIRE(ldc >= D && (ldc % 4) == 0 && ldg >= 3 * D && (ldg % 4) == 0, "dx_attention_bwd: bad leading dimensions");
   DX_REQUIRE(((uintptr_t)dctx % 16) == 0 && ((uintptr_t)dqkv % 16) == 0, "dx_attention_bwd: pointers must be 16-byte aligned");
   DX_REQUIRE(p_drop >= 0.f && p_drop < 1.f, "dx_attention_bwd: dropout p out of range");
+  DX_REQUIRE(!keep || (bf16 && ((uintptr_t)keep % 16) == 0), "dx_attention_bwd: keep bits need the 16-bit operand mode and 16-byte alignment");
   hipStream_t s = (hipStream_t)stream;
   const long items = (long)B * N * H;
   if (!bf16)
     hipLaunchKernelGGL(attn_delta_kernel, dim3((int)std::min<long>((items + 3) / 4, 8192)), dim3(256), 0, s, dctx, ctx, ldc, delta, B, N, H);
   AttnBwdArgs a{qkv, ld, dctx, ldc, lse, delta, lens, dqkv, ldg, B, N, H, D, seed, (uint32_t)lrintf(p_drop * 65536.f), 1.f / (1.f - p_drop), ctx, delta, seed_offset, order, 0};
   a.xcd_map = (H * B) % 8 == 0;
+  a.keep = a.thresh ? (const uint16_t*)keep : nullptr;
   dx_prof_begin(DX_PROF_ATTN_BWD, s);
   if (bf16) {
     const dim3 grid(dx_cdiv(N, 64), H, B);
+#define DX_ATTN_BWD2(QT_, OT_, CT_, K_)                                                                \
+    hipLaunchKernelGGL((attn_bwd_dq_bf16_kernel<QT_, OT_, CT_, K_>), grid, dim3(256), 0, s, a);        \
+    hipLaunchKernelGGL((attn_bwd_dkv_bf16_kernel<QT_, OT_, CT_, K_>), grid, dim3(256), 0, s, a);
 #define DX_ATTN_BWD(QT_, OT_)                                                                          \
-    if (ctx_bf16) {                                                                                    \
-      hipLaunchKernelGGL((attn_bwd_dq_bf16_kernel<QT_, OT_, dx_h16>), grid, dim3(256), 0, s, a);       \
-      hipLaunchKernelGGL((attn_bwd_dkv_bf16_kernel<QT_, OT_, dx_h16>), grid, dim3(256), 0, s, a);      \
-    } else {                                                                                           \
-      hipLaunchKernelGGL((attn_bwd_dq_bf16_kernel<QT_, OT_, float>), grid, dim3(256), 0, s, a);        \
-      hipLaunchKernelGGL((attn_bwd_dkv_bf16_kernel<QT_, OT_, float>), grid, dim3(256), 0, s, a);       \
-    }
+    if (ctx_bf16 && a.keep) { DX_ATTN_BWD2(QT_, OT_, dx_h16, true) }                                   \
+    else if (ctx_bf16) { DX_ATTN_BWD2(QT_, OT_, dx_h16, false) }                                       \
+    else if (a.keep) { DX_ATTN_BWD2(QT_, OT_, float, true) }                                           \
+    else { DX_ATTN_BWD2(QT_, OT_, float, false) }
     if (qkv_bf16 && dqkv_bf16) { DX_ATTN_BWD(dx_h16, dx_h16) }
     else if (qkv_bf16) { DX_ATTN_BWD(dx_h16, float) }
     else if (dqkv_bf16) { DX_ATTN_BWD(float, dx_h16) }
     else { DX_ATTN_BWD(float, float) }
 #undef DX_ATTN_BWD
+#undef DX_ATTN_BWD2
   } else if (split) {
     if constexpr (kSplitBuild) {
       static bool configured = false;
diff --git a/ubisoft_laforge_daft_exprt_amd/csrc/dx_common.h b/ubisoft_laforge_daft_exprt_amd/csrc/dx_common.h
--- a/ubisoft_laforge_daft_exprt_amd/csrc/dx_common.h
+++ b/ubisoft_laforge_daft_exprt_amd/csrc/dx_common.h
@@ -123,6 +123,28 @@
   x[0] = dx_keep_lo(lo, thresh, x[0], alt); x[1] = dx_keep_hi(lo, thresh, x[1], alt);
   x[2] = dx_keep_lo(hi, thresh, x[2], alt); x[3] = dx_keep_hi(hi, thresh, x[3], alt);
 }
+__device__ __forceinline__ void dx_keep4_rec(uint64_t r, uint32_t thresh, float x[4], float alt, uint32_t& bits) {
+  const uint32_t lo = (uint32_t)r, hi = (uint32_t)(r >> 32);
+#define DX_KEEP_REC(W, SEL, X)                                                                                                        \
+  asm("v_cmp_ge_u16_sdwa vcc, %2, %3 src0_sel:" SEL " src1_sel:WORD_0\n\tv_cndmask_b32_e32 %0, %4, %0, vcc\n\t"                      \
+      "v_addc_co_u32_e32 %1, vcc, %1, %1, vcc" : "+v"(X), "+v"(bits) : "v"(W), "v"(thresh), "v"(alt) : "vcc")
+  DX_KEEP_REC(lo, "WORD_0", x[0]); DX_KEEP_REC(lo, "WORD_1", x[1]); DX_KEEP_REC(hi, "WORD_0", x[2]); DX_KEEP_REC(hi, "WORD_1", x[3]);
+#undef DX_KEEP_REC
+}
+__device__ __forceinline__ void dx_keep4_replay(uint32_t& bits, float x[4], float alt) {
+#pragma unroll
+  for (int i = 0; i < 4; ++i)
+    asm("v_add_co_u32_e32 %1, vcc, %1, %1\n\tv_cndmask_b32_e32 %0, %2, %0, vcc" : "+v"(x[i]), "+v"(bits) : "v"(alt) : "vcc");
+}
+#define DX_KEEP2_BIT15(SEL)                                                                                                          \
+  asm("v_cmp_ge_u16_sdwa vcc, %2, %3 src0_sel:" SEL " src1_sel:WORD_0\n\tv_cndmask_b32_e32 %0, 0, %0, vcc\n\tv_cndmask_b32_e32 %1, %4, %1, vcc" \
+      : "+v"(x), "+v"(y) : "v"(w), "v"(0x8000u), "v"(alt) : "vcc")
+template <int HI>
+__device__ __forceinline__ void dx_keep2_bit15(uint32_t w, float& x, float& y, float alt) {
+  if constexpr (HI) DX_KEEP2_BIT15("WORD_1");
+  else DX_KEEP2_BIT15("WORD_0");
+}
+#undef DX_KEEP2_BIT15
 __device__ __forceinline__ void dx_dropout_scale4(uint64_t seed, uint64_t elem0, uint32_t thresh16, float inv_keep, float out[4]) {
   uint64_t r = dx_rand64(seed, elem0 >> 2);
 #pragma unroll
diff --git a/ubisoft_laforge_daft_exprt_amd/csrc/dx_f16_names.h b/ubisoft_laforge_daft_exprt_amd/csrc/dx_f16_names.h
--- a/ubisoft_laforge_daft_exprt_amd/csrc/dx_f16_names.h
+++ b/ubisoft_laforge_daft_exprt_amd/csrc/dx_f16_names.h
@@ -2,8 +2,11 @@
 #define dx_accent_sum dx_accent_sum_f16
 #define dx_add_pos dx_add_pos_f16
 #define dx_attention_bwd dx_attention_bwd_f16
+#define dx_attention_bwd_keep dx_attention_bwd_keep_f16
 #define dx_attention_fwd dx_attention_fwd_f16
+#define dx_attention_fwd_keep dx_attention_fwd_keep_f16
 #define dx_attention_proj_ln_fwd dx_attention_proj_ln_fwd_f16
+#define dx_attention_proj_ln_fwd_keep dx_attention_proj_ln_fwd_keep_f16
 #define dx_channel_affine dx_channel_affine_f16
 #define dx_colsum dx_colsum_f16
 #define dx_condition_prosody dx_condition_prosody_f16
diff --git a/ubisoft_laforge_daft_exprt_amd/functional.py b/ubisoft_laforge_daft_exprt_amd/functional.py
--- a/ubisoft_laforge_daft_exprt_amd/functional.py
+++ b/ubisoft_laforge_daft_exprt_amd/functional.py
@@ -132,12 +132,14 @@
             ops.conv_gemm(x, packs['in'], in_b, lens=L, halo=0, out_dtype=hd, prec=prec)
         so = rt.seed_offset
         sh = ops.gemm_shadow(prec)
+        keep = ops.keep_bits(qkv, heads) if p_attn > 0 and any(ctx.needs_input_grad) and ops._half(prec) else None
         if ops.attn_proj_ln_applies(qkv, heads, packs['out'], prec):
             att, lse, z1, y1, mean1, rstd1, *rest = ops.attn_proj_ln_fwd(qkv, lens.i32, heads, s_attn, p_attn, packs['out'], out_b, x, ln1_w, ln1_b, None,
-                                                                         seed_pre=s_ln1, p_pre=p_attn, shadow=sh, seed_offset=so, prec=prec)
+                                                                         seed_pre=s_ln1, p_pre=p_attn, shadow=sh, seed_offset=so, prec=prec,
+                                                                         keep=keep)
             y1g = rest[0] if sh else y1
         else:
-            att, lse = ops.attention_fwd(qkv, lens.i32, heads, s_attn, p_attn, prec=prec, seed_offset=so, ctx_dtype=hd)
+            att, lse = ops.attention_fwd(qkv, lens.i32, heads, s_attn, p_attn, prec=prec, seed_offset=so, ctx_dtype=hd, keep=keep)
             z1 = ops.conv_gemm(att, packs['out'], out_b, lens=L, halo=0, prec=prec)
             ln1 = ops.ln_fwd(z1, x, ln1_w, ln1_b, None, lens.i32, seed_pre=s_ln1, p_pre=p_attn, shadow=sh, seed_offset=so, prec=prec)
             y1, mean1, rstd1 = ln1[:3]
@@ -163,6 +165,7 @@
         ctx.drop = (p_attn, p_conv, s_attn, s_ln1, s_ln2)
         ctx.prec, ctx.sink, ctx.fused, ctx.seed_offset = prec, rt.sink, fused, so
         ctx.hmask = hmask
+        ctx.keep = keep
         if qkv_next is not None:
             ctx.mark_non_differentiable(qkv_next)
         ctx.set_materialize_grads(False)
@@ -211,7 +214,7 @@
         dout_w, dout_b = ops.conv_wgrad(dproj, att, packs['out'], L, 0, arena=arena, w_sink=g('out_w'), b_sink=g('out_b'), prec=prec, defer=True)
         if datt is None:
             datt = ops.conv_gemm(dproj, packs['out'], None, transpose=True, lens=L, halo=0, prec=prec, out_dtype=att.dtype)
-        dqkv = ops.attention_bwd(qkv, att, datt, lse, L, ctx.heads, s_attn, p_attn, out_dtype=qkv.dtype, prec=prec, seed_offset=so)
+        dqkv = ops.attention_bwd(qkv, att, datt, lse, L, ctx.heads, s_attn, p_attn, out_dtype=qkv.dtype, prec=prec, seed_offset=so, keep=ctx.keep)
         din_w, din_b = ops.conv_wgrad(dqkv, x, packs['in'], L, 0, arena=arena, w_sink=g('in_w'), b_sink=g('in_b'), prec=prec, defer=True)
         dx = ops.conv_gemm(dqkv, packs['in'], None, transpose=True, out=dz1, accumulate=True, lens=L, halo=0, prec=prec)
         return (dx, dfilm, None, None, None, None,
diff --git a/ubisoft_laforge_daft_exprt_amd/ops.py b/ubisoft_laforge_daft_exprt_amd/ops.py
--- a/ubisoft_laforge_daft_exprt_amd/ops.py
+++ b/ubisoft_laforge_daft_exprt_amd/ops.py
@@ -478,19 +478,29 @@
     return order
 
 
-def attention_fwd(qkv, lens, heads, seed, p_drop, prec=None, seed_offset=None, ctx_dtype=torch.float32, order=None):
+def keep_bits(qkv, heads):
+    B, N, _ = qkv.shape
+    T = -(-N // 64)
+    return torch.empty(B * heads * T * T * 256, dtype=torch.int16, device=qkv.device)
+
+
+def attention_fwd(qkv, lens, heads, seed, p_drop, prec=None, seed_offset=None, ctx_dtype=torch.float32, order=None, keep=None):
     B, N, D3 = qkv.shape
     D = D3 // 3
     ctx = torch.empty(B, N, D, dtype=ctx_dtype, device=qkv.device)
     lse = torch.empty(B, heads, N, dtype=torch.float32, device=qkv.device)
     prec = prec or DEFAULT.precision
     _check_h16(prec, qkv, ctx)
-    _fn('dx_attention_fwd', prec)(_p(qkv), _rows(qkv), _p(lens), _p(ctx), D, _p(lse), B, N, heads, D, seed, _p(seed_offset), float(p_drop),
-                           _mode(prec), _is_bf16(qkv), _is_bf16(ctx), _p(order), _stream())
+    args = (_p(qkv), _rows(qkv), _p(lens), _p(ctx), D, _p(lse), B, N, heads, D, seed, _p(seed_offset), float(p_drop), _mode(prec), _is_bf16(qkv),
+            _is_bf16(ctx), _p(order))
+    if keep is None:
+        _fn('dx_attention_fwd', prec)(*args, _stream())
+    else:
+        _fn('dx_attention_fwd_keep', prec)(*args, _p(keep), _stream())
     return ctx, lse
 
 
-def attention_bwd(qkv, ctx, dctx, lse, lens, heads, seed, p_drop, out_dtype=torch.float32, prec=None, seed_offset=None, order=None):
+def attention_bwd(qkv, ctx, dctx, lse, lens, heads, seed, p_drop, out_dtype=torch.float32, prec=None, seed_offset=None, order=None, keep=None):
     B, N, D3 = qkv.shape
     D = D3 // 3
     if dctx.dtype != ctx.dtype:
@@ -498,9 +508,12 @@
     dqkv = torch.empty(B, N, D3, dtype=out_dtype, device=qkv.device)
     delta = torch.empty(B, heads, N, dtype=torch.float32, device=qkv.device)
     prec = prec or DEFAULT.precision
-    _fn('dx_attention_bwd', prec)(_p(qkv), _rows(qkv), _p(ctx), _p(dctx), _rows(dctx), _p(lse), _p(delta), _p(lens), _p(dqkv), _rows(dqkv),
-                           B, N, heads, D, seed, _p(seed_offset), float(p_drop), _mode(prec), _is_bf16(qkv), _is_bf16(dqkv), _is_bf16(ctx),
-                           _p(order), _stream())
+    args = (_p(qkv), _rows(qkv), _p(ctx), _p(dctx), _rows(dctx), _p(lse), _p(delta), _p(lens), _p(dqkv), _rows(dqkv), B, N, heads, D, seed,
+            _p(seed_offset), float(p_drop), _mode(prec), _is_bf16(qkv), _is_bf16(dqkv), _is_bf16(ctx), _p(order))
+    if keep is None:
+        _fn('dx_attention_bwd', prec)(*args, _stream())
+    else:
+        _fn('dx_attention_bwd_keep', prec)(*args, _p(keep), _stream())
     return dqkv
 
 
@@ -526,7 +539,7 @@
 
 
 def attn_proj_ln_fwd(qkv, lens, heads, seed, p_drop, pack: PackedWeight, proj_bias, res, w, b, film, *, seed_pre=0, p_pre=0.0, shadow=False,
-                     seed_offset=None, prec=None):
+                     seed_offset=None, prec=None, keep=None):
     B, N, D3 = qkv.shape
     D = D3 // 3
     prec = prec or pack.rt.precision
@@ -541,9 +554,12 @@
     rstd = torch.empty(B, N, dtype=torch.float32, device=qkv.device)
     img = pack.image(prec)
     _log(pack, ('gemm', B * N, N, pack.cin, pack.cout, 1))
-    _fn('dx_attention_proj_ln_fwd', prec)(_p(qkv), _rows(qkv), _p(lens), _p(ctx), D, _p(lse), B, N, heads, D, seed, _p(seed_offset), float(p_drop),
-                                          _p(img.fwd), _p(proj_bias), _p(z), _p(res), _p(w), _p(b), _p(film), 0 if film is None else film.stride(0),
-                                          _p(y), _p(mean), _p(rstd), seed_pre, float(p_pre), _p(y_h), _stream())
+    args = (_p(qkv), _rows(qkv), _p(lens), _p(ctx), D, _p(lse), B, N, heads, D, seed, _p(seed_offset), float(p_drop), _p(img.fwd), _p(proj_bias),
+            _p(z), _p(res), _p(w), _p(b), _p(film), 0 if film is None else film.stride(0), _p(y), _p(mean), _p(rstd), seed_pre, float(p_pre), _p(y_h))
+    if keep is None:
+        _fn('dx_attention_proj_ln_fwd', prec)(*args, _stream())
+    else:
+        _fn('dx_attention_proj_ln_fwd_keep', prec)(*args, _p(keep), _stream())
     return (ctx, lse, z, y, mean, rstd, y_h) if shadow else (ctx, lse, z, y, mean, rstd)
 
 
diff --git a/ubisoft_laforge_daft_exprt_amd/profiling.py b/ubisoft_laforge_daft_exprt_amd/profiling.py
--- a/ubisoft_laforge_daft_exprt_amd/profiling.py
+++ b/ubisoft_laforge_daft_exprt_amd/profiling.py
@@ -41,6 +41,10 @@
     has = lambda k: bool(g(k))
     if name.endswith('_f16'):
         name = name[:-4]
+    if name.startswith('dx_attention') and name.endswith('_keep'):
+        keep = geom.pairs(a['B'], a['N']) * a['H'] / 8 if has('keep') else 0
+        label, bound, flops, byt = price(name[:-5], a, geom)
+        return label, bound, flops, (None if byt is None else byt + keep)
     if name == 'dx_conv_gemm':
         rows = geom.rows(a['B'], a['N'], has('lens'))
         xb, yb, ab = (2 if a['x_bf16'] else 4), (2 if a['y_bf16'] else 4), (2 if a['aux_bf16'] else 4)
```

New measurement: 4.978 million (median of 6 runs). 2.1% higher.
